# qgallouedec/deep_rl

Measured on NVIDIA B200. Metric: PPO env-steps/sec (rollout+update) CartPole-v1, higher is better.
Workload: dtype bf16

## Files before the change

### deep_rl_b200/_lib.py

```python
from __future__ import annotations

import ctypes as C
import os

import torch

from . import build as _build

_LIB = None

u8p, i32p, u32p, u64p, f32p, f64p = (C.c_void_p,) * 6


class EnvT(C.Structure):
    _fields_ = [("kind", C.c_int32), ("num_envs", C.c_int32), ("seed", C.c_uint64), ("env_gid0", C.c_uint32),
                ("max_episode_steps", C.c_int32), ("state", C.c_void_p), ("elapsed", C.c_void_p),
                ("ep_ret", C.c_void_p), ("ep_len", C.c_void_p)]


class EpLogT(C.Structure):
    _fields_ = [("count", C.c_void_p), ("sum_ret", C.c_void_p), ("sum_len", C.c_void_p), ("entries", C.c_void_p),
                ("cap", C.c_uint32)]


class NetT(C.Structure):
    _fields_ = [("obs_dim", C.c_int32), ("hidden", C.c_int32), ("num_actions", C.c_int32), ("obs_stride", C.c_int32)]


class RolloutBufT(C.Structure):
    _fields_ = [("obs", C.c_void_p), ("act", C.c_void_p), ("logp", C.c_void_p), ("val", C.c_void_p),
                ("rew", C.c_void_p), ("done", C.c_void_p), ("logits", C.c_void_p)]


class CommT(C.Structure):
    _fields_ = [("world", C.c_int32), ("rank", C.c_int32), ("peer", C.c_void_p * 8), ("seq", C.c_uint32),
                ("error_flag", C.c_void_p)]


class CtrlT(C.Structure):
    _fields_ = [("env_step", C.c_uint64), ("epoch_ctr", C.c_uint32), ("comm_seq", C.c_uint32), ("adam_step", C.c_int64),
                ("neg_step_size", C.c_float * 64), ("bc2_sqrt", C.c_float * 64)]


class PpoCoefT(C.Structure):
    _fields_ = [("clip_coef", C.c_float), ("ent_coef", C.c_float), ("vf_coef", C.c_float)]


SIGNATURES = {
    "drl_abi_version": (C.c_int, []),
    "drl_last_error": (C.c_char_p, []),
    "drl_env_obs_dim": (C.c_int, [C.c_int32]),
    "drl_env_num_actions": (C.c_int, [C.c_int32]),
    "drl_env_obs_stride": (C.c_int, [C.c_int32]),
    "drl_param_count": (C.c_int64, [C.POINTER(NetT)]),
    "drl_packed_count": (C.c_int64, [C.POINTER(NetT)]),
    "drl_record_width": (C.c_int, [C.POINTER(NetT)]),
    "drl_workspace_bytes": (C.c_size_t, [C.POINTER(NetT)]),
    "drl_env_reset": (C.c_int, [C.POINTER(EnvT), f32p, C.c_void_p]),
    "drl_env_observe": (C.c_int, [C.POINTER(EnvT), f32p, C.c_void_p]),
    "drl_env_step": (C.c_int, [C.POINTER(EnvT), C.c_uint64, i32p, f32p, f32p, u8p, C.POINTER(EpLogT), C.c_void_p]),
    "drl_pack_params": (C.c_int, [C.POINTER(NetT), f32p, f32p, C.c_void_p]),
    "drl_policy_forward": (C.c_int, [C.POINTER(NetT), f32p, f32p, C.c_int64, f32p, f32p, C.c_void_p]),
    "drl_sample": (C.c_int, [f32p, C.c_int64, C.c_int32, C.c_uint64, C.c_uint32, C.c_uint64, i32p, f32p, C.c_void_p]),
    "drl_rollout": (C.c_int, [C.POINTER(EnvT), C.POINTER(NetT), f32p, C.c_int32, C.c_uint64, C.POINTER(RolloutBufT),
                              C.POINTER(EpLogT), C.c_uint32, C.c_void_p]),
    "drl_gae": (C.c_int, [C.POINTER(RolloutBufT), C.POINTER(NetT), C.c_int32, C.c_int32, C.c_float, C.c_float, f32p,
                          f32p, f32p, C.c_void_p]),
    "drl_explained_variance": (C.c_int, [f32p, f32p, C.c_int64, f32p, C.c_void_p, C.c_size_t, C.c_void_p]),
    "drl_permutation": (C.c_int, [u32p, C.c_uint32, C.c_uint64, C.c_uint32, C.c_uint32, C.c_void_p]),
    "drl_adv_stats": (C.c_int, [C.POINTER(NetT), f32p, u32p, C.c_uint32, C.c_uint32, f32p, C.c_void_p, C.c_size_t,
                                C.c_void_p]),
    "drl_adv_stats_perm": (C.c_int, [C.POINTER(NetT), f32p, C.c_uint32, C.c_uint32, C.c_uint64, C.c_uint32, C.c_uint32, f32p,
                                     C.c_void_p, C.c_size_t, C.c_void_p]),
    "drl_ppo_minibatch_grad": (C.c_int, [C.POINTER(NetT), f32p, f32p, u32p, C.c_uint32, C.c_uint32, f32p,
                                         C.POINTER(PpoCoefT), f32p, f32p, C.c_void_p, C.c_size_t, C.c_uint32, C.c_void_p]),
    "drl_ppo_minibatch_update": (C.c_int, [C.POINTER(NetT), f32p, f32p, u32p, C.c_uint32, C.c_uint32, f32p, C.POINTER(PpoCoefT),
                                           f32p, f32p, f32p, f32p, C.c_int64, C.c_double, C.c_double, C.c_double, C.c_double,
                                           C.c_double, f32p, f32p, C.c_void_p, C.c_size_t, C.c_uint32, C.c_int32, C.c_void_p]),
    "drl_ppo_minibatch_update_dist": (C.c_int, [C.POINTER(NetT), f32p, f32p, u32p, C.c_uint32, C.c_uint32, f32p, C.POINTER(PpoCoefT),
                                                f32p, f32p, f32p, f32p, C.c_int64, C.c_double, C.c_double, C.c_double, C.c_double,
                                                C.c_double, f32p, f32p, C.c_void_p, C.c_size_t, C.c_uint32, C.POINTER(CommT),
                                                C.c_int32, C.c_void_p]),
    "drl_ctrl_set": (C.c_int, [C.c_void_p, C.c_uint64, C.c_uint32, C.c_uint32, C.c_int64, C.c_int32, C.c_double, C.c_double, C.c_double,
                               C.c_void_p]),
    "drl_rollout_ctl": (C.c_int, [C.POINTER(EnvT), C.POINTER(NetT), f32p, C.c_int32, C.c_void_p, C.POINTER(RolloutBufT),
                                  C.POINTER(EpLogT), C.c_uint32, C.c_void_p]),
    "drl_permutation_ctl": (C.c_int, [u32p, C.c_uint32, C.c_uint64, C.c_void_p, C.c_uint32, C.c_uint32, C.c_void_p]),
    "drl_adv_stats_perm_ctl": (C.c_int, [C.POINTER(NetT), f32p, C.c_uint32, C.c_uint32, C.c_uint64, C.c_void_p, C.c_uint32, C.c_uint32,
                                         f32p, C.c_void_p, C.c_size_t, C.c_void_p]),
    "drl_ppo_minibatch_update_ctl": (C.c_int, [C.POINTER(NetT), f32p, f32p, u32p, C.c_uint32, C.c_uint32, f32p, C.POINTER(PpoCoefT),
                                               f32p, f32p, f32p, f32p, C.c_void_p, C.c_int32, C.c_double, C.c_double, C.c_double,
                                               C.c_double, f32p, f32p, C.c_void_p, C.c_size_t, C.c_uint32, C.POINTER(CommT),
                                               C.c_int32, C.c_void_p]),
    "drl_comm_bytes": (C.c_size_t, [C.POINTER(NetT)]),
    "drl_comm_alloc": (C.c_int, [C.c_size_t, C.POINTER(C.c_void_p), C.c_void_p]),
    "drl_comm_open": (C.c_int, [C.c_void_p, C.POINTER(C.c_void_p)]),
    "drl_comm_close": (C.c_int, [C.c_void_p]),
    "drl_comm_free": (C.c_int, [C.c_void_p]),
    "drl_replay_sample_uniform": (C.c_int, [u32p, C.c_uint32, C.c_uint32, C.c_uint64, C.c_uint64, C.c_void_p]),
    "drl_replay_gather": (C.c_int, [f32p, i32p, f32p, u8p, u32p, C.c_uint32, C.c_int32, f32p, f32p, i32p, f32p, u8p, C.c_void_p]),
    "drl_replay_scratch_bytes": (C.c_size_t, [C.c_uint32]),
    "drl_replay_sample_priority": (C.c_int, [f32p, C.c_uint32, C.c_float, C.c_uint32, C.c_uint64, C.c_uint64, u32p, f32p, C.c_void_p,
                                             C.c_size_t, C.c_void_p]),
    "drl_replay_update_priorities": (C.c_int, [f32p, u32p, f32p, C.c_uint32, f32p, C.c_void_p]),
    "drl_reinforce_param_count": (C.c_int, []),
    "drl_reinforce_episodes": (C.c_int, [C.POINTER(EnvT), f32p, C.c_int32, C.c_uint64, f32p, u8p, f32p, u8p, i32p, u32p, C.POINTER(EpLogT),
                                         C.c_void_p]),
    "drl_reinforce_grad": (C.c_int, [f32p, f32p, u8p, f32p, i32p, u32p, C.c_int32, C.c_uint64, C.c_uint32, C.c_uint64, C.c_float, f32p, f32p,
                                     f32p, f32p, C.c_void_p]),
    "drl_adam_step": (C.c_int, [f32p, f32p, f32p, f32p, C.c_int64, C.c_int64, C.c_double, C.c_double, C.c_double, C.c_double, C.c_void_p]),
    "drl_selftest_umma": (C.c_int, [C.c_int32, C.c_int32, f32p, f32p, f32p, C.c_void_p]),
    "drl_selftest_tanh": (C.c_int, [f32p, f32p, C.c_int64, C.c_void_p]),
    "drl_clip_adam": (C.c_int, [C.POINTER(NetT), f32p, f32p, f32p, f32p, C.c_int64, C.c_double, C.c_double, C.c_double,
                                C.c_double, C.c_double, C.c_double, f32p, f32p, C.c_void_p]),
}


class DrlError(RuntimeError):
    pass


def lib_path() -> str:
    return _build.SO


ABI_VERSION = 2


def lib() -> C.CDLL:
    global _LIB
    if _LIB is None:
        path = _build.build_locked()
        L = C.CDLL(path)
        for name, (res, args) in SIGNATURES.items():
            fn = getattr(L, name)
            fn.restype, fn.argtypes = res, args
        if L.drl_abi_version() != ABI_VERSION:
            raise DrlError(f"libdrl_b200 ABI version {L.drl_abi_version()} != {ABI_VERSION}")
        _LIB = L
    return _LIB


def check(rc: int) -> None:
    if rc != 0:
        raise DrlError(f"libdrl_b200 error {rc}: {lib().drl_last_error().decode()}")


def require_cuda() -> None:
    if not torch.cuda.is_available():
        raise DrlError("deep_rl_b200 needs a CUDA device (B200, sm_100a); there is no CPU fallback")


def ptr(t) -> int:
    return 0 if t is None else t.data_ptr()


def stream_ptr() -> int:
    return torch.cuda.current_stream().cuda_stream
```

### deep_rl_b200/csrc/drl_pack.cuh

```cuda
#pragma once
#include <cuda_bf16.h>

#include "drl_common.cuh"

namespace drl {

int check_net(const drl_net_t* net);

template <int O, int A>
__device__ __forceinline__ void packed_store(float* __restrict__ packed, int i, float v) {
    using P = Packed<O, A>;
    const int net = i >= P::C_ACTOR ? 1 : 0;
    int r = i - net * P::C_ACTOR;
    if (r < H * O) {
        const int o = r / O, k = r % O;
        packed[P::W1T + (net * O + k) * H + perm_pos(o)] = v;
        packed[P::TC_W1 + (net * H + o) * P::OW + k] = __bfloat162float(__float2bfloat16_rn(v));
        __nv_bfloat16* w1b = reinterpret_cast<__nv_bfloat16*>(packed + P::TC_W1B) + net * (2 * H * 8);
        w1b[o * 8 + k] = __float2bfloat16_rn(v);
        w1b[H * 8 + o * 8 + k] = __float2bfloat16_rn(v);
        return;
    }
    r -= H * O;
    if (r < H) {
        packed[P::B1 + net * H + perm_pos(r)] = v;
        packed[P::TC_B1 + net * H + r] = __bfloat162float(__float2bfloat16_rn(v));
        reinterpret_cast<__nv_bfloat16*>(packed + P::TC_W1B)[net * (2 * H * 8) + r * 8 + O] = __float2bfloat16_rn(v);
        return;
    }
    r -= H;
    if (r < H * H) {
        const int o = r / H, k = r % H;
        packed[P::W2T + (net * H + k) * H + perm_pos(o)] = v;
        packed[P::W2P + (net * H + o) * H + perm_pos(k)] = v;
        unsigned char* tc = reinterpret_cast<unsigned char*>(packed + P::TC_W2);
        const int off = net * (H * H * 2) + o * 128 + ((((k >> 3) ^ (o & 7)) << 4)) + (k & 7) * 2;
        *reinterpret_cast<__nv_bfloat16*>(tc + off) = __float2bfloat16_rn(v);
        return;
    }
    r -= H * H;
    if (r < H) {
        packed[P::B2 + net * H + perm_pos(r)] = v;
        packed[P::TC_B2 + net * H + r] = v;
        return;
    }
    r -= H;
    const int nout = net == 0 ? A : 1;
    if (r < nout * H) {
        const int a = r / H, k = r % H;
        packed[P::W4 + (net * A + a) * H + perm_pos(k)] = v;
        packed[P::TC_W4 + (net == 0 ? a : A) * H + k] = v;
        return;
    }
    r -= nout * H;
    packed[P::B4 + net * A + r] = v;
    packed[P::TC_B4 + (net == 0 ? r : A)] = v;
}

constexpr int MAX_GRAD_CTAS = 160;
constexpr int MAX_MINIBATCHES = 16;
constexpr int STAT_PARTS = 512;
constexpr int LOSS_TERMS = 8;

struct WorkspaceLayout {
    size_t counters, stat_partials, cta_sumsq, loss_partials, grad_partials, debug, ev_partials, stage, total;
    int ppad;
};
inline WorkspaceLayout workspace_layout(int64_t P, int hidden = 64) {
    WorkspaceLayout w;
    w.ppad = (int)((P + 3) / 4 * 4);
    w.counters = 0;
    w.stat_partials = 64;
    w.cta_sumsq = w.stat_partials + sizeof(double) * MAX_MINIBATCHES * STAT_PARTS * 2;
    w.ev_partials = w.cta_sumsq + sizeof(double) * 1024;
    w.loss_partials = w.ev_partials + sizeof(double) * STAT_PARTS * 4;
    w.grad_partials = w.loss_partials + sizeof(float) * MAX_GRAD_CTAS * LOSS_TERMS;
    w.debug = (w.grad_partials + sizeof(float) * (size_t)MAX_GRAD_CTAS * w.ppad + 1023) / 1024 * 1024;
    w.stage = w.debug + 4096;
    w.total = w.stage + (hidden == 256 ? (size_t)2 * 2 * 4096 * 65536 : 0);
    return w;
}
inline size_t workspace_bytes_for(int64_t P, int hidden = 64) { return workspace_layout(P, hidden).total; }

}
```

### deep_rl_b200/csrc/drl_update.cuh

```cuda
#pragma once
#include "drl_common.cuh"

namespace drl {

constexpr int DRL_MAX_STEPS_PER_LAUNCH = 8;

struct AdamArgs {
    float* params; const float* grad; float* m; float* v; float* packed; float* norm_out;
    int P;
    float grad_scale, max_norm, beta2, om_beta1, om_beta2, eps, neg_step_size, bc2_sqrt;
};

struct TailArgs {
    int enabled;
    AdamArgs a;
    float* grad_out; float* loss_terms_out;
    double* cta_sumsq;
    uint32_t* ctr;
    int world, rank;
    unsigned char* peer[DRL_MAX_RANKS];
    uint32_t seq;
    int* error_flag;
    const drl_ctrl_t* ctrl;
    int ordinal;
    int nsteps;
    float neg_step_size_s[DRL_MAX_STEPS_PER_LAUNCH], bc2_sqrt_s[DRL_MAX_STEPS_PER_LAUNCH];
};

constexpr int FLAG_CTAS = 160;
struct CommLayout {
    size_t xgrad[2], flags[2], rank_stride, total;
};
__host__ __device__ inline CommLayout comm_layout(int64_t P) {
    CommLayout c;
    const size_t g = ((size_t)P * 4 + 255) / 256 * 256;
    c.rank_stride = g;
    c.xgrad[0] = 0; c.xgrad[1] = (size_t)DRL_MAX_RANKS * g;
    c.flags[0] = 2 * (size_t)DRL_MAX_RANKS * g; c.flags[1] = c.flags[0] + sizeof(uint32_t) * DRL_MAX_RANKS * FLAG_CTAS;
    c.total = c.flags[1] + sizeof(uint32_t) * DRL_MAX_RANKS * FLAG_CTAS;
    return c;
}

struct GradArgs {
    const float* packed;
    const float* rec;
    const uint32_t* idx;
    uint32_t mb_start, mb_count;
    const float* adv_stats;
    float clip_coef, ent_coef, vf_coef;
    float* grad_part;
    float* loss_part;
    int ppad;
    long long* dbg;
    TailArgs tail;
};

int launch_grad_reduce(const GradArgs& g, int grid, int P, float* grad_out, float* loss_terms_out, cudaStream_t st);

int launch_grad_tc(const drl_net_t* net, const GradArgs& g, int P, float* grad_out, float* loss_terms_out, cudaStream_t st,
                   int* grid_out = nullptr);
int launch_grad_tc_fused(const drl_net_t* net, GradArgs& g, cudaStream_t st);

}
```

### deep_rl_b200/csrc/gae_ops.cu

```cuda
#include "drl_pack.cuh"

namespace drl {

template <int OP, int RW>
__global__ void __launch_bounds__(128) gae_kernel(const float* __restrict__ rew, const uint8_t* __restrict__ done,
                                                   const float* __restrict__ val, const float* __restrict__ obs,
                                                   const uint8_t* __restrict__ act, const float* __restrict__ logp,
                                                   int T, int N, float gamma, float lam, float* __restrict__ adv,
                                                   float* __restrict__ ret, float* __restrict__ rec) {
    const int n = blockIdx.x * blockDim.x + threadIdx.x;
    if (n >= N) return;
    float last = 0.0f;
    float v1 = val[(size_t)T * N + n];
    adv[(size_t)T * N + n] = 0.0f;
    ret[(size_t)T * N + n] = 0.0f + v1;
    constexpr int GB = 8;
    for (int tb = T - 1; tb >= 0; tb -= GB) {
        float r_[GB], v_[GB], lp_[GB];
        uint8_t d_[GB], a_[GB];
        float4 o_[GB][OP / 4];
#pragma unroll
        for (int j = 0; j < GB; ++j) {
            const int t = tb - j;
            if (t >= 0) {
                const size_t i0 = (size_t)t * N + n, i1 = i0 + N;
                d_[j] = done[i1];
                r_[j] = rew[i1];
                v_[j] = val[i0];
                if (rec != nullptr) {
                    lp_[j] = logp[i0];
                    a_[j] = act[i0];
                    const float4* o4 = reinterpret_cast<const float4*>(obs + i0 * OP);
#pragma unroll
                    for (int q = 0; q < OP / 4; ++q) o_[j][q] = o4[q];
                }
            }
        }
#pragma unroll
        for (int j = 0; j < GB; ++j) {
            const int t = tb - j;
            if (t >= 0) {
                const size_t i0 = (size_t)t * N + n;
                const float d = (float)d_[j];
                const float v0 = v_[j];
                const float nd = 1.0f - d;
                const float a = gamma * nd;
                const float ll = lam * last;
                const float b = v1 + ll;
                const float c = a * b;
                const float dd = r_[j] + c;
                const float ad = dd - v0;
                adv[i0] = ad;
                ret[i0] = ad + v0;
                if (rec != nullptr) {
                    float4* r4 = reinterpret_cast<float4*>(rec + i0 * RW);
                    r4[0] = o_[j][0];
                    if (RW == 16) {
                        r4[1] = o_[j][OP / 4 - 1];
                        r4[2] = make_float4(0.f, 0.f, 0.f, 0.f);
                    }
                    r4[RW / 4 - 1] = make_float4(lp_[j], ad, v0, __int_as_float((int)a_[j]));
                }
                last = ad;
                v1 = v0;
            }
        }
    }
}

constexpr int PERM_ROUNDS = 6;

__device__ __forceinline__ uint32_t fmix32(uint32_t h) {
    h ^= h >> 16; h *= 0x85EBCA6Bu; h ^= h >> 13; h *= 0xC2B2AE35u; h ^= h >> 16;
    return h;
}

__device__ __forceinline__ uint32_t perm_index(uint32_t i, uint32_t B, uint32_t a, uint32_t b, const uint32_t (&keys)[8]) {
    uint32_t x = i;
    do {
        uint32_t lb = a, rb = b;
        uint32_t L = x >> rb, R = x & ((1u << rb) - 1u);
#pragma unroll
        for (uint32_t r = 0; r < PERM_ROUNDS; ++r) {
            const uint32_t nR = L ^ (fmix32(R ^ keys[r]) & ((1u << lb) - 1u));
            L = R;
            R = nR;
            const uint32_t t = lb; lb = rb; rb = t;
        }
        x = (L << rb) | R;
    } while (x >= B);
    return x;
}

__global__ void __launch_bounds__(256) permutation_kernel(uint32_t* __restrict__ idx, uint32_t B, uint32_t a, uint32_t b,
                                                           uint64_t seed, uint32_t epoch_ctr, uint32_t rank,
                                                           const drl_ctrl_t* __restrict__ ctrl) {
    if (ctrl != nullptr) epoch_ctr += ctrl->epoch_ctr;
    const uint4 k0 = philox_seeded(seed, epoch_ctr, rank, 0u, TAG_PERM);
    const uint4 k1 = philox_seeded(seed, epoch_ctr, rank, 1u, TAG_PERM);
    const uint32_t keys[8] = {k0.x, k0.y, k0.z, k0.w, k1.x, k1.y, k1.z, k1.w};
    const uint32_t stride = gridDim.x * blockDim.x;
    for (uint32_t i = blockIdx.x * blockDim.x + threadIdx.x; i < B; i += stride)
        idx[i] = perm_index(i, B, a, b, keys);
}

template <int RW>
__global__ void __launch_bounds__(256) adv_stats_kernel(const float* __restrict__ rec, const uint32_t* __restrict__ idx,
                                                         uint32_t B, uint32_t mb_size, float* __restrict__ stats_out,
                                                         double* __restrict__ partials, uint32_t* __restrict__ counter) {
    const uint32_t mb = blockIdx.y, part = blockIdx.x, nmb = gridDim.y, nparts = gridDim.x;
    const uint32_t lo = mb * mb_size;
    const uint32_t hi = min(B, lo + mb_size);
    double s = 0.0, ss = 0.0;
    const uint32_t step = nparts * 256u;
    uint32_t i = lo + part * 256u + threadIdx.x;
    for (; i + 3u * step < hi; i += 4u * step) {
        uint32_t sx[4];
#pragma unroll
        for (int j = 0; j < 4; ++j) sx[j] = idx ? __ldg(idx + i + j * step) : i + j * step;
        float av[4];
#pragma unroll
        for (int j = 0; j < 4; ++j) av[j] = __ldg(rec + (size_t)sx[j] * RW + (RW - 3));
#pragma unroll
        for (int j = 0; j < 4; ++j) { const double a = (double)av[j]; s += a; ss = fma(a, a, ss); }
    }
    for (; i < hi; i += step) {
        const uint32_t sidx = idx ? idx[i] : i;
        const double a = (double)rec[(size_t)sidx * RW + (RW - 3)];
        s += a;
        ss = fma(a, a, ss);
    }
    __shared__ double sh[2][8];
    __shared__ bool is_last;
    s = warp_sum(s);
    ss = warp_sum(ss);
    const int warp = threadIdx.x >> 5, lane = threadIdx.x & 31;
    if (lane == 0) { sh[0][warp] = s; sh[1][warp] = ss; }
    __syncthreads();
    if (threadIdx.x == 0) {
        double ts = 0.0, tss = 0.0;
        for (int w = 0; w < 8; ++w) { ts += sh[0][w]; tss += sh[1][w]; }
        partials[((size_t)mb * STAT_PARTS + part) * 2 + 0] = ts;
        partials[((size_t)mb * STAT_PARTS + part) * 2 + 1] = tss;
        __threadfence();
        const uint32_t done = atomicAdd(counter, 1u);
        is_last = (done == nmb * nparts - 1);
    }
    __syncthreads();
    if (is_last && threadIdx.x < nmb) {
        __threadfence();
        const uint32_t k = threadIdx.x;
        double ts = 0.0, tss = 0.0;
        for (uint32_t p = 0; p < nparts; ++p) {
            ts += __ldcg(&partials[((size_t)k * STAT_PARTS + p) * 2 + 0]);
            tss += __ldcg(&partials[((size_t)k * STAT_PARTS + p) * 2 + 1]);
        }
        const uint32_t klo = k * mb_size, khi = min(B, klo + mb_size);
        const double cnt = (double)(khi - klo);
        const double mean = ts / cnt;
        const double var = (tss - ts * mean) / (cnt - 1.0);
        stats_out[2 * k + 0] = (float)mean;
        stats_out[2 * k + 1] = (float)sqrt(var > 0.0 ? var : 0.0);
        if (k == 0) *counter = 0;
    }
}

constexpr int STATS_MAX_MB = 8;

__device__ __forceinline__ uint32_t perm_position(uint32_t s, uint32_t B, uint32_t a, uint32_t b, const uint32_t (&keys)[8]) {
    uint32_t x = s;
    do {
        uint32_t lb = a, rb = b;
        uint32_t L = x >> rb, R = x & ((1u << rb) - 1u);
#pragma unroll
        for (int r = PERM_ROUNDS - 1; r >= 0; --r) {
            const uint32_t t = lb; lb = rb; rb = t;
            const uint32_t R0 = L;
            const uint32_t L0 = R ^ (fmix32(R0 ^ keys[r]) & ((1u << lb) - 1u));
            L = L0; R = R0;
        }
        x = (L << rb) | R;
    } while (x >= B);
    return x;
}

__global__ void __launch_bounds__(256) adv_stats_perm_kernel(const float* __restrict__ adv, uint32_t B, uint32_t mb_size, uint32_t nmb,
                                                              uint32_t a, uint32_t b, uint64_t seed, uint32_t epoch_ctr, uint32_t rank,
                                                              float* __restrict__ stats_out, double* __restrict__ partials,
                                                              uint32_t* __restrict__ counter, const drl_ctrl_t* __restrict__ ctrl) {
    if (ctrl != nullptr) epoch_ctr += ctrl->epoch_ctr;
    const uint4 k0 = philox_seeded(seed, epoch_ctr, rank, 0u, TAG_PERM);
    const uint4 k1 = philox_seeded(seed, epoch_ctr, rank, 1u, TAG_PERM);
    const uint32_t keys[8] = {k0.x, k0.y, k0.z, k0.w, k1.x, k1.y, k1.z, k1.w};
    double sm_[STATS_MAX_MB], ss_[STATS_MAX_MB];
#pragma unroll
    for (int m = 0; m < STATS_MAX_MB; ++m) { sm_[m] = 0.0; ss_[m] = 0.0; }
    const uint32_t stride = gridDim.x * blockDim.x;
    for (uint32_t s = blockIdx.x * blockDim.x + threadIdx.x; s < B; s += stride) {
        const double v = (double)__ldg(adv + s);
        const uint32_t mb = perm_position(s, B, a, b, keys) / mb_size;
#pragma unroll
        for (int m = 0; m < STATS_MAX_MB; ++m)
            if (mb == (uint32_t)m) { sm_[m] += v; ss_[m] = fma(v, v, ss_[m]); }
    }
    __shared__ double sh[2][STATS_MAX_MB][8];
    __shared__ bool is_last;
    const int warp = threadIdx.x >> 5, lane = threadIdx.x & 31;
#pragma unroll
    for (int m = 0; m < STATS_MAX_MB; ++m) {
        const double t0 = warp_sum(sm_[m]), t1 = warp_sum(ss_[m]);
        if (lane == 0) { sh[0][m][warp] = t0; sh[1][m][warp] = t1; }
    }
    __syncthreads();
    if (threadIdx.x < 2 * STATS_MAX_MB) {
        const int which = threadIdx.x / STATS_MAX_MB, m = threadIdx.x % STATS_MAX_MB;
        double t = 0.0;
        for (int w = 0; w < 8; ++w) t += sh[which][m][w];
        partials[((size_t)m * STAT_PARTS + blockIdx.x) * 2 + which] = t;
    }
    __threadfence();
    __syncthreads();
    if (threadIdx.x == 0) {
        const uint32_t done = atomicAdd(counter, 1u);
        is_last = (done == gridDim.x - 1);
    }
    __syncthreads();
    if (is_last) {
        __threadfence();
        const uint32_t k = threadIdx.x >> 5;
        if (k < nmb) {
            double ts = 0.0, tss = 0.0;
            for (uint32_t p = threadIdx.x & 31; p < gridDim.x; p += 32) {
                ts += __ldcg(&partials[((size_t)k * STAT_PARTS + p) * 2 + 0]);
                tss += __ldcg(&partials[((size_t)k * STAT_PARTS + p) * 2 + 1]);
            }
            ts = warp_sum(ts);
            tss = warp_sum(tss);
            if ((threadIdx.x & 31) == 0) {
                const uint32_t klo = k * mb_size, khi = min(B, klo + mb_size);
                const double cnt = (double)(khi - klo);
                const double mean = ts / cnt;
                const double var = (tss - ts * mean) / (cnt - 1.0);
                stats_out[2 * k + 0] = (float)mean;
                stats_out[2 * k + 1] = (float)sqrt(var > 0.0 ? var : 0.0);
            }
        }
        __syncthreads();
        if (threadIdx.x == 0) *counter = 0;
    }
}

__global__ void __launch_bounds__(256) explained_variance_kernel(const float* __restrict__ values, const float* __restrict__ returns,
                                                                  int64_t n, float* __restrict__ out, double* __restrict__ partials,
                                                                  uint32_t* __restrict__ counter) {
    double acc[4] = {0.0, 0.0, 0.0, 0.0};
    const int64_t stride = (int64_t)gridDim.x * blockDim.x;
    for (int64_t i = (int64_t)blockIdx.x * blockDim.x + threadIdx.x; i < n; i += stride) {
        const float yf = __ldg(values + i), rf = __ldg(returns + i);
        const double y = (double)yf, d = (double)(yf - rf);
        acc[0] += y; acc[1] = fma(y, y, acc[1]); acc[2] += d; acc[3] = fma(d, d, acc[3]);
    }
    __shared__ double sh[4][8];
    __shared__ bool is_last;
    const int warp = threadIdx.x >> 5, lane = threadIdx.x & 31;
#pragma unroll
    for (int q = 0; q < 4; ++q) {
        const double t = warp_sum(acc[q]);
        if (lane == 0) sh[q][warp] = t;
    }
    __syncthreads();
    if (threadIdx.x < 4) {
        double t = 0.0;
        for (int w = 0; w < 8; ++w) t += sh[threadIdx.x][w];
        partials[(size_t)blockIdx.x * 4 + threadIdx.x] = t;
    }
    __threadfence();
    __syncthreads();
    if (threadIdx.x == 0) is_last = atomicAdd(counter, 1u) == gridDim.x - 1;
    __syncthreads();
    if (is_last && threadIdx.x < 32) {
        __threadfence();
        double t[4] = {0.0, 0.0, 0.0, 0.0};
        for (uint32_t p = threadIdx.x; p < gridDim.x; p += 32)
#pragma unroll
            for (int q = 0; q < 4; ++q) t[q] += __ldcg(&partials[(size_t)p * 4 + q]);
#pragma unroll
        for (int q = 0; q < 4; ++q) t[q] = warp_sum(t[q]);
        if (threadIdx.x == 0) {
            const double cnt = (double)n;
            const double var_y = (t[1] - t[0] * (t[0] / cnt)) / (cnt - 1.0);
            const double var_d = (t[3] - t[2] * (t[2] / cnt)) / (cnt - 1.0);
            out[0] = var_y == 0.0 ? __int_as_float(0x7FC00000) : (float)(1.0 - var_d / var_y);
            *counter = 0;
        }
    }
}

}

using namespace drl;

extern "C" {

int drl_gae(const drl_rollout_buf_t* buf, const drl_net_t* net, int32_t T, int32_t N, float gamma, float gae_lambda,
            float* adv_out, float* ret_out, float* rec_out, void* stream) {
    int rc = check_net(net);
    if (rc != DRL_OK) return rc;
    DRL_REQUIRE(buf && buf->rew && buf->done && buf->val && adv_out && ret_out, "drl_gae: NULL pointer");
    DRL_REQUIRE(T > 0 && N > 0, "drl_gae: T=%d N=%d", T, N);
    DRL_REQUIRE(rec_out == nullptr || (buf->obs && buf->act && buf->logp), "drl_gae: record packing needs obs/act/logp");
    const int blocks = (N + 127) / 128;
    cudaStream_t st = as_stream(stream);
    if (net->obs_stride == 4)
        gae_kernel<4, 8><<<blocks, 128, 0, st>>>(buf->rew, buf->done, buf->val, buf->obs, buf->act, buf->logp, T, N, gamma,
                                                gae_lambda, adv_out, ret_out, rec_out);
    else
        gae_kernel<8, 16><<<blocks, 128, 0, st>>>(buf->rew, buf->done, buf->val, buf->obs, buf->act, buf->logp, T, N, gamma,
                                                 gae_lambda, adv_out, ret_out, rec_out);
    DRL_LAUNCH_CHECK("gae_kernel");
    return DRL_OK;
}

int drl_explained_variance(const float* values, const float* returns, int64_t n, float* out, void* workspace,
                           size_t workspace_bytes, void* stream) {
    DRL_REQUIRE(values && returns && out && workspace, "drl_explained_variance: NULL pointer");
    DRL_REQUIRE(n >= 2, "drl_explained_variance: n=%lld", (long long)n);
    const WorkspaceLayout w = workspace_layout(0);
    DRL_REQUIRE(workspace_bytes >= w.total, "drl_explained_variance: workspace %zu < %zu bytes", workspace_bytes, w.total);
    uint32_t* counter = reinterpret_cast<uint32_t*>((char*)workspace + w.counters) + 12;
    double* partials = reinterpret_cast<double*>((char*)workspace + w.ev_partials);
    int64_t blocks = (n + 4095) / 4096;
    if (blocks > STAT_PARTS) blocks = STAT_PARTS;
    explained_variance_kernel<<<(int)blocks, 256, 0, as_stream(stream)>>>(values, returns, n, out, partials, counter);
    DRL_LAUNCH_CHECK("explained_variance_kernel");
    return DRL_OK;
}

static int permutation_impl(uint32_t* idx_out, uint32_t B, uint64_t seed, uint32_t epoch_ctr, uint32_t rank, void* stream,
                            const drl_ctrl_t* ctrl) {
    DRL_REQUIRE(idx_out, "drl_permutation: idx_out is NULL");
    DRL_REQUIRE(B > 0 && B <= 0x80000000u, "drl_permutation: B=%u out of range", B);
    DRL_REQUIRE(rank < (1u << 24), "drl_permutation: rank=%u out of range", rank);
    uint32_t k = 2;
    while (k < 32 && (1ull << k) < (unsigned long long)B) ++k;
    const uint32_t a = k / 2, b = k - a;
    long long blocks = ((long long)B + 2047) / 2048;
    const long long cap = (long long)sm_count() * 16;
    if (blocks > cap) blocks = cap;
    permutation_kernel<<<(int)blocks, 256, 0, as_stream(stream)>>>(idx_out, B, a, b, seed, epoch_ctr, rank, ctrl);
    DRL_LAUNCH_CHECK("permutation_kernel");
    return DRL_OK;
}
int drl_permutation(uint32_t* idx_out, uint32_t B, uint64_t seed, uint32_t epoch_ctr, uint32_t rank, void* stream) {
    return permutation_impl(idx_out, B, seed, epoch_ctr, rank, stream, nullptr);
}
int drl_permutation_ctl(uint32_t* idx_out, uint32_t B, uint64_t seed, const drl_ctrl_t* ctrl, uint32_t epoch_off, uint32_t rank,
                        void* stream) {
    DRL_REQUIRE(ctrl != nullptr, "drl_permutation_ctl: ctrl is NULL");
    return permutation_impl(idx_out, B, seed, epoch_off, rank, stream, ctrl);
}

int drl_adv_stats(const drl_net_t* net, const float* rec, const uint32_t* idx, uint32_t B, uint32_t mb_size,
                  float* stats_out, void* workspace, size_t workspace_bytes, void* stream) {
    int rc = check_net(net);
    if (rc != DRL_OK) return rc;
    DRL_REQUIRE(rec && stats_out && workspace, "drl_adv_stats: NULL pointer");
    DRL_REQUIRE(B > 0 && mb_size > 0, "drl_adv_stats: B=%u mb_size=%u", B, mb_size);
    const uint32_t nmb = (B + mb_size - 1) / mb_size;
    DRL_REQUIRE(nmb <= (uint32_t)MAX_MINIBATCHES, "drl_adv_stats: %u minibatches > %d", nmb, MAX_MINIBATCHES);
    const WorkspaceLayout w = workspace_layout(drl_param_count(net));
    DRL_REQUIRE(workspace_bytes >= w.total, "drl_adv_stats: workspace %zu < %zu bytes", workspace_bytes, w.total);
    uint32_t* counter = reinterpret_cast<uint32_t*>((char*)workspace + w.counters);
    double* partials = reinterpret_cast<double*>((char*)workspace + w.stat_partials);
    uint32_t nparts = (mb_size + 4095u) / 4096u;
    if (nparts > (uint32_t)STAT_PARTS) nparts = STAT_PARTS;
    if (nparts == 0) nparts = 1;
    dim3 grid(nparts, nmb);
    if (net->obs_dim <= 4) adv_stats_kernel<8><<<grid, 256, 0, as_stream(stream)>>>(rec, idx, B, mb_size, stats_out, partials, counter);
    else adv_stats_kernel<16><<<grid, 256, 0, as_stream(stream)>>>(rec, idx, B, mb_size, stats_out, partials, counter);
    DRL_LAUNCH_CHECK("adv_stats_kernel");
    return DRL_OK;
}

static int adv_stats_perm_impl(const drl_net_t* net, const float* adv, uint32_t B, uint32_t mb_size, uint64_t seed, uint32_t epoch_ctr,
                               uint32_t rank, float* stats_out, void* workspace, size_t workspace_bytes, void* stream,
                               const drl_ctrl_t* ctrl) {
    int rc = check_net(net);
    if (rc != DRL_OK) return rc;
    DRL_REQUIRE(adv && stats_out && workspace, "drl_adv_stats_perm: NULL pointer");
    DRL_REQUIRE(B > 0 && mb_size > 0 && B <= 0x80000000u, "drl_adv_stats_perm: B=%u mb_size=%u", B, mb_size);
    const uint32_t nmb = (B + mb_size - 1) / mb_size;
    if (nmb > (uint32_t)STATS_MAX_MB) { set_error("drl_adv_stats_perm: %u minibatches > %d (use drl_adv_stats)", nmb, STATS_MAX_MB); return DRL_ERR_UNSUPPORTED; }
    const WorkspaceLayout w = workspace_layout(drl_param_count(net));
    DRL_REQUIRE(workspace_bytes >= w.total, "drl_adv_stats_perm: workspace %zu < %zu bytes", workspace_bytes, w.total);
    uint32_t* counter = reinterpret_cast<uint32_t*>((char*)workspace + w.counters);
    double* partials = reinterpret_cast<double*>((char*)workspace + w.stat_partials);
    uint32_t k = 2;
    while (k < 32 && (1ull << k) < (unsigned long long)B) ++k;
    uint32_t blocks = (B + 2047u) / 2048u;
    if (blocks > (uint32_t)STAT_PARTS) blocks = STAT_PARTS;
    adv_stats_perm_kernel<<<blocks, 256, 0, as_stream(stream)>>>(adv, B, mb_size, nmb, k / 2, k - k / 2, seed, epoch_ctr, rank,
                                                                 stats_out, partials, counter, ctrl);
    DRL_LAUNCH_CHECK("adv_stats_perm_kernel");
    return DRL_OK;
}
int drl_adv_stats_perm(const drl_net_t* net, const float* adv, uint32_t B, uint32_t mb_size, uint64_t seed, uint32_t epoch_ctr,
                       uint32_t rank, float* stats_out, void* workspace, size_t workspace_bytes, void* stream) {
    return adv_stats_perm_impl(net, adv, B, mb_size, seed, epoch_ctr, rank, stats_out, workspace, workspace_bytes, stream, nullptr);
}
int drl_adv_stats_perm_ctl(const drl_net_t* net, const float* adv, uint32_t B, uint32_t mb_size, uint64_t seed, const drl_ctrl_t* ctrl,
                           uint32_t epoch_off, uint32_t rank, float* stats_out, void* workspace, size_t workspace_bytes, void* stream) {
    DRL_REQUIRE(ctrl != nullptr, "drl_adv_stats_perm_ctl: ctrl is NULL");
    return adv_stats_perm_impl(net, adv, B, mb_size, seed, epoch_off, rank, stats_out, workspace, workspace_bytes, stream, ctrl);
}

}
```

### deep_rl_b200/csrc/update_tc.cu

```cuda
#include "drl_pack.cuh"
#include "drl_tc_common.cuh"
#include "drl_update.cuh"

namespace drl {

constexpr uint32_t C_ZF = 0, C_DH = 128, C_W2 = 256, C_B2 = 384, C_W4 = 400, C_W1 = 416, TC_COLS = 512;

template <int O, int A>
struct TcSmem {
    using P = Packed<O, A>;
    static constexpr int W_BYTES = (P::TC_END - P::TC_W2) * 4;
    static constexpr int OFF_W = 0;
    static constexpr int OFF_H1 = (OFF_W + W_BYTES + 1023) / 1024 * 1024;
    static constexpr int OFF_H2 = OFF_H1 + 65536;
    static constexpr int OFF_DZ = OFF_H2 + 32768;
    static constexpr int OFF_DZ1 = OFF_DZ + 32768;
    static constexpr int OFF_OBS = OFF_DZ1 + 32768;
    static constexpr int OFF_DOUT = OFF_OBS + 12288;
    static constexpr int OFF_SCAL = OFF_DOUT + 4096;
    static constexpr int OFF_BAR = OFF_SCAL + 3 * 2048;
    static constexpr int OFF_XCH = OFF_BAR + 128;
    static constexpr int OFF_RED = OFF_XCH + 2 * 2 * 4 * 128 * 4;
    static constexpr int OFF_CTX = OFF_RED + 16 * 12 * 4;
    static constexpr int TOTAL = OFF_CTX + 512 + 1024;
    static_assert(TOTAL <= 232448, "exceeds the 227 KB of shared memory a CTA can opt in to");
};

#ifdef DRL_TC_STAMPS
#define TC_STAMP(ev) do { if (g.dbg != nullptr && blockIdx.x == 0 && lane == 0 && k < 12 && (warp == 0 || warp == TC_COMPUTE / 32)) g.dbg[(warp == 0 ? 0 : 256) + k * 16 + (ev)] = clock64(); } while (0)
#define TC_KSTAMP(n) do { if (g.dbg != nullptr && blockIdx.x == 0 && tid == 0) g.dbg[256 + ((n) >> 3) * 16 + 8 + ((n) & 7)] = clock64(); } while (0)
#else
#define TC_STAMP(ev) do { } while (0)
#define TC_KSTAMP(n) do { } while (0)
#endif

enum : uint32_t { BAR_FWD = 1, BAR_BWD = 2, BAR_W1 = 3, BAR_PAIR0 = 4, BAR_L1 = 12 };

constexpr int GRAD_TC_BLOCK = TC_THREADS + 32;
constexpr int RING = 3;

__device__ __forceinline__ uint32_t tc_sample_index(const GradArgs& g, uint32_t mb_start, uint32_t mb_count, uint32_t tile, uint32_t ntiles, int r) {
    const uint32_t pos = tile * TC_TILE + (uint32_t)r;
    if (tile >= ntiles || pos >= mb_count) return 0xFFFFFFFFu;
    const uint32_t i = mb_start + pos;
    return g.idx ? __ldg(g.idx + i) : i;
}

struct TailCtx {
    TailArgs tl;
    float* grad_part; float* loss_part; float* packed; long long* dbg;
    int ppad; uint32_t mb_count; float ent_coef, vf_coef;
};
static_assert(sizeof(TailCtx) <= 512, "TailCtx block");

template <int O, int A>
__device__ __noinline__ void tc_tail_step(const TailCtx* cx, uint32_t s, uint32_t nsteps, unsigned char* sm, uint64_t* bars) {
    using P = Packed<O, A>;
    using S = TcSmem<O, A>;
    const int tid = threadIdx.x, warp = tid >> 5, lane = tid & 31;
    const struct { long long* dbg; } g = {cx->dbg};
    (void)g;
    constexpr uint32_t BAR_TAIL = 13;
    const TailArgs& tl = cx->tl;
    const AdamArgs& ad = tl.a;
    const int PP = ad.P;
    float neg_step_size = tl.neg_step_size_s[s], bc2_sqrt = tl.bc2_sqrt_s[s];
    uint32_t seq = tl.seq + s;
    if (tl.ctrl != nullptr) {
        neg_step_size = tl.ctrl->neg_step_size[tl.ordinal + s];
        bc2_sqrt = tl.ctrl->bc2_sqrt[tl.ordinal + s];
        seq = tl.ctrl->comm_seq + (uint32_t)(tl.ordinal + s) + 1u;
    }
    float* const loss_terms_out = tl.loss_terms_out != nullptr ? tl.loss_terms_out + LOSS_TERMS * s : nullptr;
    const uint32_t bar_target = (s + 1u) * gridDim.x;
    const int nparts = gridDim.x;
    float* tred = reinterpret_cast<float*>(sm + S::OFF_H1);
    double* dred = reinterpret_cast<double*>(sm + S::OFF_H1 + 4096);
    float* sbc = reinterpret_cast<float*>(sm + S::OFF_H1 + 8192);
    auto grid_barrier = [&](uint32_t* ctr) {
        named_bar_sync(BAR_TAIL, TC_COMPUTE);
        if (tid == 0) {
            asm volatile("red.release.gpu.global.add.u32 [%0], 1;" ::"l"(ctr) : "memory");
            uint32_t seen;
            do {
                asm volatile("ld.acquire.gpu.global.u32 %0, [%1];" : "=r"(seen) : "l"(ctr) : "memory");
            } while (seen < bar_target);
        }
        named_bar_sync(BAR_TAIL, TC_COMPUTE);
    };
    grid_barrier(tl.ctr + 0);
    TC_KSTAMP(6);
    const int chunk = (PP + nparts - 1) / nparts;
    const int p_lo = blockIdx.x * chunk, p_hi = min(PP, p_lo + chunk);
    const int pl = tid & 63, sl = tid >> 6;
    const bool multi = tl.world > 1;
    const CommLayout cl = comm_layout(PP);
    const uint32_t gen = seq & 1u;
    double sq = 0.0;
    for (int p0 = p_lo; p0 < p_hi; p0 += 64) {
        const int p = p0 + pl;
        float a0 = 0.f, a1 = 0.f, a2 = 0.f, a3 = 0.f;
        if (p < p_hi) {
            static_assert(MAX_GRAD_CTAS <= 160, "fold is unrolled for at most 160 partials");
            float pv[20];
#pragma unroll
            for (int j = 0; j < 20; ++j) {
                const int c = sl + 8 * j;
                pv[j] = c < nparts ? __ldcg(cx->grad_part + (size_t)c * cx->ppad + p) : 0.0f;
            }
            bool rest = false;
#pragma unroll
            for (int gq = 0; gq < 5; ++gq) {
                const int c = sl + 32 * gq;
                if (!rest && c + 24 < nparts) {
                    a0 += pv[4 * gq]; a1 += pv[4 * gq + 1]; a2 += pv[4 * gq + 2]; a3 += pv[4 * gq + 3];
                } else {
                    rest = true;
#pragma unroll
                    for (int q = 0; q < 4; ++q)
                        if (c + 8 * q < nparts) a0 += pv[4 * gq + q];
                }
            }
        }
        tred[sl * 64 + pl] = (a0 + a1) + (a2 + a3);
        named_bar_sync(BAR_TAIL, TC_COMPUTE);
        if (sl == 0 && p < p_hi) {
            float t = tred[pl];
#pragma unroll
            for (int y = 1; y < 8; ++y) t += tred[y * 64 + pl];
            if (multi) {
                for (int rk = 0; rk < tl.world; ++rk)
                    reinterpret_cast<float*>(tl.peer[rk] + cl.xgrad[gen] + (size_t)tl.rank * cl.rank_stride)[p] = t;
            } else {
                tl.grad_out[p] = t;
                const double gs = (double)(t * ad.grad_scale);
                sq = fma(gs, gs, sq);
            }
        }
        named_bar_sync(BAR_TAIL, TC_COMPUTE);
    }
    TC_KSTAMP(7);
    if (multi) {
        if (sl == 0) __threadfence_system();
        named_bar_sync(BAR_TAIL, TC_COMPUTE);
        if (tid < tl.world) {
            __threadfence_system();
            *reinterpret_cast<volatile uint32_t*>(tl.peer[tid] + cl.flags[gen] + sizeof(uint32_t) * (tl.rank * FLAG_CTAS + blockIdx.x)) = seq;
            const volatile uint32_t* f = reinterpret_cast<const volatile uint32_t*>(tl.peer[tl.rank] + cl.flags[gen] +
                                                                                    sizeof(uint32_t) * (tid * FLAG_CTAS + blockIdx.x));
            const long long t0 = clock64();
            while (*f < seq) {
                if (clock64() - t0 > 40000000000ll) {
                    if (tl.error_flag) { *reinterpret_cast<volatile int*>(tl.error_flag) = 1; __threadfence(); }
                    break;
                }
            }
            __threadfence_system();
        }
        named_bar_sync(BAR_TAIL, TC_COMPUTE);
        const float* mine = reinterpret_cast<const float*>(tl.peer[tl.rank] + cl.xgrad[gen]);
        for (int p = p_lo + tid; p < p_hi; p += TC_COMPUTE) {
            float t = 0.0f;
            for (int rk = 0; rk < tl.world; ++rk)
                t += __ldcg(mine + (size_t)rk * (cl.rank_stride / sizeof(float)) + p);
            tl.grad_out[p] = t;
            const double gs = (double)(t * ad.grad_scale);
            sq = fma(gs, gs, sq);
        }
    }
    sq = warp_sum(sq);
    if (lane == 0) dred[warp] = sq;
    named_bar_sync(BAR_TAIL, TC_COMPUTE);
    if (tid == 0) {
        double t = 0.0;
        for (int wv = 0; wv < TC_COMPUTE / 32; ++wv) t += dred[wv];
        tl.cta_sumsq[blockIdx.x] = t;
    }
    TC_KSTAMP(8);
    const int p_first = p_lo + tid;
    float pre_m = 0.f, pre_v = 0.f, pre_w = 0.f;
    if (p_first < p_hi) { pre_m = ad.m[p_first]; pre_v = ad.v[p_first]; pre_w = ad.params[p_first]; }
    grid_barrier(tl.ctr + 2);
    TC_KSTAMP(9);
    if (warp == 0) {
        double tot = 0.0;
        for (int i = lane; i < nparts; i += 32) tot += __ldcg(tl.cta_sumsq + i);
        tot = warp_sum(tot);
        if (lane == 0) {
            const float norm = (float)sqrt(tot);
            const float cf = ad.max_norm / (norm + 1e-6f);
            sbc[0] = cf < 1.0f ? cf : 1.0f;
            if (blockIdx.x == 0 && ad.norm_out) *ad.norm_out = norm;
        }
    } else if (blockIdx.x == 0 && warp >= 1 && warp <= 5 && loss_terms_out != nullptr) {
        float t = 0.f;
        for (int c = lane; c < nparts; c += 32) t += __ldcg(cx->loss_part + c * LOSS_TERMS + (warp - 1));
        t = warp_sum(t);
        if (lane == 0) sbc[4 + warp - 1] = t;
    }
    named_bar_sync(BAR_TAIL, TC_COMPUTE);
    const float coef = sbc[0];
    const bool peer_lost = multi && tl.error_flag != nullptr && *reinterpret_cast<volatile int*>(tl.error_flag) != 0;
    for (int p = p_lo + tid; p < p_hi && !peer_lost; p += TC_COMPUTE) {
        const float gsc = (__ldcg(tl.grad_out + p) * ad.grad_scale) * coef;
        float m, v, wgt;
        if (p == p_first) { m = pre_m; v = pre_v; wgt = pre_w; }
        else { m = ad.m[p]; v = ad.v[p]; wgt = ad.params[p]; }
        m = m + ad.om_beta1 * (gsc - m);
        v = v * ad.beta2 + (ad.om_beta2 * gsc) * gsc;
        const float denom = sqrtf(v) / bc2_sqrt + ad.eps;
        wgt = wgt + (neg_step_size * m) / denom;
        ad.m[p] = m; ad.v[p] = v; ad.params[p] = wgt;
        if (ad.packed != nullptr) packed_store<O, A>(ad.packed, p, wgt);
    }
    TC_KSTAMP(10);
    if (blockIdx.x == 0 && tid == 0 && loss_terms_out != nullptr) {
        const float inv = 1.0f / (float)cx->mb_count;
        const float pg = sbc[4] * inv, vl = 0.5f * sbc[5] * inv, en = sbc[6] * inv;
        loss_terms_out[0] = pg - cx->ent_coef * en + vl * cx->vf_coef;
        loss_terms_out[1] = pg; loss_terms_out[2] = vl; loss_terms_out[3] = en;
        loss_terms_out[4] = sbc[7] * inv; loss_terms_out[5] = sbc[8] * inv;
        loss_terms_out[6] = 0.0f; loss_terms_out[7] = 0.0f;
    }
    if (s + 1 < nsteps) {
        grid_barrier(tl.ctr + 1);
        if (tid == 0) {
            asm volatile("fence.proxy.async;" ::: "memory");
            mbar_expect_tx(bars, (uint32_t)S::W_BYTES);
            const char* src = reinterpret_cast<const char*>(cx->packed + P::TC_W2);
            for (uint32_t off = 0; off < (uint32_t)S::W_BYTES; off += 16384u) {
                const uint32_t nb = (uint32_t)S::W_BYTES - off < 16384u ? (uint32_t)S::W_BYTES - off : 16384u;
                bulk_g2s(sm + S::OFF_W + off, src + off, nb, bars);
            }
        }
    } else if (tid == 0) {
        __threadfence();
        if (atomicAdd(tl.ctr + 3, 1u) == gridDim.x - 1) { tl.ctr[0] = 0u; tl.ctr[1] = 0u; tl.ctr[2] = 0u; tl.ctr[3] = 0u; }
    }
}

template <int O, int A, int OP, int RW>
__global__ void __launch_bounds__(GRAD_TC_BLOCK, 1) ppo_grad_tc_kernel(const __grid_constant__ GradArgs g) {
    using P = Packed<O, A>;
    using S = TcSmem<O, A>;
    constexpr int OW = P::OW;
    extern __shared__ unsigned char smem_raw[];
    unsigned char* sm = smem_raw + ((1024u - (smem_u32(smem_raw) & 1023u)) & 1023u);
    unsigned char* tW2 = sm + S::OFF_W;
    const float* sW1 = reinterpret_cast<const float*>(sm + S::OFF_W + 2 * H * H * 2);
    const float* sB1 = sW1 + 2 * H * OW;
    const float* sB2 = sB1 + 2 * H;
    const float* sW4 = sB2 + 2 * H;
    const float* sB4 = sW4 + (A + 1) * H;
    unsigned char* tW1B = reinterpret_cast<unsigned char*>(const_cast<float*>(sB4 + 4));
    unsigned char* tH1 = sm + S::OFF_H1;
    unsigned char* tH2 = sm + S::OFF_H2;
    unsigned char* tDZ = sm + S::OFF_DZ;
    unsigned char* tDZ1 = sm + S::OFF_DZ1;
    unsigned char* tOBS = sm + S::OFF_OBS;
    unsigned char* tDOUT = sm + S::OFF_DOUT;
    uint4* sSCAL = reinterpret_cast<uint4*>(sm + S::OFF_SCAL);
    uint64_t* bars = reinterpret_cast<uint64_t*>(sm + S::OFF_BAR);
    uint64_t* ring_full = bars + 7;
    uint64_t* ring_empty = bars + 7 + RING;
    uint32_t* slot = reinterpret_cast<uint32_t*>(bars + 7 + 2 * RING);
    float* xch = reinterpret_cast<float*>(sm + S::OFF_XCH);
    float* red = reinterpret_cast<float*>(sm + S::OFF_RED);

    const int tid = threadIdx.x, warp = tid >> 5, lane = tid & 31;
    const bool is_mma_warp = warp == TC_COMPUTE / 32;
    const bool is_loader_warp = warp == TC_COMPUTE / 32 + 1;
    const int rw = warp & 3, half = (warp >> 2) & 1, net = (warp >> 3) & 1;
    const int r = rw * 32 + lane;
    const int u0 = half * HU;
    const uint32_t nsteps = g.tail.enabled ? (uint32_t)g.tail.nsteps : 1u;
    const uint32_t ntiles = (g.mb_count + TC_TILE - 1) / TC_TILE;
    const uint32_t nmy = (ntiles - blockIdx.x + gridDim.x - 1) / gridDim.x;

    TC_KSTAMP(0);
    if (tid == 0) {
#pragma unroll
        for (int i = 0; i < 7; ++i) mbar_init(bars + i, 1);
#pragma unroll
        for (int i = 0; i < RING; ++i) { mbar_init(ring_full + i, 32); mbar_init(ring_empty + i, 1); }
        mbar_fence_init();
    }
    if (warp == 1) umma::tmem_alloc(slot, TC_COLS);
    if (tid == 64 && g.tail.enabled) {
        TailCtx* c = reinterpret_cast<TailCtx*>(sm + S::OFF_CTX);
        c->tl = g.tail;
        c->grad_part = g.grad_part; c->loss_part = g.loss_part; c->packed = const_cast<float*>(g.packed); c->dbg = g.dbg;
        c->ppad = g.ppad; c->mb_count = g.mb_count; c->ent_coef = g.ent_coef; c->vf_coef = g.vf_coef;
    }
    umma::fence_before_sync();
    __syncthreads();
    umma::fence_after_sync();
    if (tid == 0) {
        mbar_expect_tx(bars, (uint32_t)S::W_BYTES);
        const char* src = reinterpret_cast<const char*>(g.packed + P::TC_W2);
        for (uint32_t off = 0; off < (uint32_t)S::W_BYTES; off += 16384u) {
            const uint32_t n = (uint32_t)S::W_BYTES - off < 16384u ? (uint32_t)S::W_BYTES - off : 16384u;
            bulk_g2s(sm + S::OFF_W + off, src + off, n, bars);
        }
    }
    const uint32_t tmem = *slot;

    if (is_loader_warp) {
        uint32_t sidx[4];
#pragma unroll
        for (int q = 0; q < 4; ++q) sidx[q] = tc_sample_index(g, g.mb_start, g.mb_count, blockIdx.x, ntiles, lane + 32 * q);
        uint32_t b = 0, use_par = 0;
        for (uint32_t jg = 0; jg < nsteps * nmy; ++jg) {
            const uint32_t j = jg % nmy;
            float4 rv[4][OP / 4 + 1];
#pragma unroll
            for (int q = 0; q < 4; ++q) {
#pragma unroll
                for (int c = 0; c <= OP / 4; ++c) rv[q][c] = make_float4(0.f, 0.f, 0.f, 0.f);
                rv[q][OP / 4].w = __int_as_float(-1);
                if (sidx[q] != 0xFFFFFFFFu) {
                    const float4* r4 = reinterpret_cast<const float4*>(g.rec + (size_t)sidx[q] * RW);
#pragma unroll
                    for (int c = 0; c < OP / 4; ++c) rv[q][c] = __ldg(r4 + c);
                    rv[q][OP / 4] = __ldg(r4 + RW / 4 - 1);
                }
            }
            if (jg + 1 < nsteps * nmy) {
                const uint32_t jn = (jg + 1) % nmy, sn = (jg + 1) / nmy;
#pragma unroll
                for (int q = 0; q < 4; ++q)
                    sidx[q] = tc_sample_index(g, g.mb_start + sn * g.mb_count, g.mb_count, blockIdx.x + jn * gridDim.x, ntiles, lane + 32 * q);
            }
            (void)j;
            if (jg >= RING) mbar_wait(ring_empty + b, use_par ^ 1u);
            unsigned char* obst = tOBS + b * 4096;
#pragma unroll
            for (int q = 0; q < 4; ++q) {
                const int row = lane + 32 * q;
                float o16[16];
#pragma unroll
                for (int i = 0; i < 16; ++i) o16[i] = 0.0f;
#pragma unroll
                for (int i = 0; i < O; ++i) {
                    const float4 v4 = rv[q][i / 4];
                    const float x = (i & 3) == 0 ? v4.x : ((i & 3) == 1 ? v4.y : ((i & 3) == 2 ? v4.z : v4.w));
                    const float hi = __bfloat162float(__float2bfloat16_rn(x));
                    o16[i] = hi;
                    o16[8 + i] = x - hi;
                }
                o16[O] = 1.0f;
                umma::store_row_ns16(obst, TC_TILE, row, o16);
                sSCAL[b * TC_TILE + row] = make_uint4(__float_as_uint(rv[q][OP / 4].x), __float_as_uint(rv[q][OP / 4].y),
                                                      __float_as_uint(rv[q][OP / 4].z), __float_as_uint(rv[q][OP / 4].w));
            }
            umma::fence_proxy_async();
            mbar_arrive(ring_full + b);
            if (++b == RING) { b = 0; use_par ^= 1u; }
        }
        __syncthreads();
        return;
    }

    if (is_mma_warp) {
        const uint32_t aW2 = smem_u32(tW2), aH1 = smem_u32(tH1), aH2 = smem_u32(tH2), aDZ = smem_u32(tDZ);
        const uint32_t aOBS = smem_u32(tOBS), aDOUT = smem_u32(tDOUT), aDZ1 = smem_u32(tDZ1);
        constexpr uint32_t ID_FWD = umma::make_idesc(128, 64, false, false);
        constexpr uint32_t ID_DH1 = umma::make_idesc(128, 64, false, true);
        constexpr uint32_t ID_W2 = umma::make_idesc(128, 128, true, true);
        constexpr uint32_t ID_N16 = umma::make_idesc(128, 16, true, true);
        const uint32_t aW1B = smem_u32(tW1B);
        constexpr uint32_t ID_L1 = umma::make_idesc(128, 64, false, false);
        auto issue_l1 = [&](uint32_t slot_b) {
            const uint32_t obsb = aOBS + slot_b * 4096;
#pragma unroll
            for (int n2 = 0; n2 < 2; ++n2)
                umma::mma(tmem + C_ZF + n2 * 64, umma::make_desc(obsb, 2048, 128, umma::LAYOUT_NONE),
                          umma::make_desc(aW1B + n2 * 2048, 1024, 128, umma::LAYOUT_NONE), ID_L1, 0u);
            umma::commit(bars + 4);
        };
        auto issue_fwd = [&](uint32_t k) {
            const uint32_t h1b = aH1 + (k & 1u) * 32768;
#pragma unroll
            for (int n2 = 0; n2 < 2; ++n2)
#pragma unroll
                for (int kb = 0; kb < 4; ++kb)
                    umma::mma(tmem + C_ZF + n2 * 64, umma::make_desc(h1b + n2 * 16384 + kb * 32, 16, 1024, umma::LAYOUT_SW128),
                              umma::make_desc(aW2 + n2 * 8192 + kb * 32, 16, 1024, umma::LAYOUT_SW128), ID_FWD, kb > 0);
            umma::commit(bars + 1);
        };
        uint32_t bn = 0, bn_par = 0;
        uint32_t bc = 0;
        for (uint32_t s = 0; s < nsteps; ++s) {
        const uint32_t kbase = s * nmy;
        mbar_wait(bars, s & 1u);
        named_bar_sync(BAR_L1, TC_THREADS);
        mbar_wait(ring_full + bn, bn_par);
        umma::fence_after_sync();
        if (umma::elect_one()) issue_l1(bn);
        __syncwarp();
        if (++bn == RING) { bn = 0; bn_par ^= 1u; }
        named_bar_sync(BAR_FWD, TC_THREADS);
        umma::fence_after_sync();
        if (umma::elect_one()) issue_fwd(kbase);
        __syncwarp();
        for (uint32_t k = 0; k < nmy; ++k) {
            const uint32_t par = (kbase + k) & 1u, acc = k > 0 ? 1u : 0u;
            const uint32_t obsb = aOBS + bc * 4096;
            if (k + 1 < nmy) {
                named_bar_sync(BAR_L1, TC_THREADS);
                mbar_wait(ring_full + bn, bn_par);
                umma::fence_after_sync();
                if (umma::elect_one()) issue_l1(bn);
                __syncwarp();
                if (++bn == RING) { bn = 0; bn_par ^= 1u; }
            }
            named_bar_sync(BAR_BWD, TC_THREADS);
            umma::fence_after_sync();
            TC_STAMP(0);
            if (umma::elect_one()) {
#pragma unroll
                for (int n2 = 0; n2 < 2; ++n2)
#pragma unroll
                    for (int kb = 0; kb < 4; ++kb)
                        umma::mma(tmem + C_DH + n2 * 64, umma::make_desc(aDZ + n2 * 16384 + kb * 32, 16, 1024, umma::LAYOUT_SW128),
                                  umma::make_desc(aW2 + n2 * 8192 + kb * 2048, 8192, 1024, umma::LAYOUT_SW128), ID_DH1, kb > 0);
                umma::commit(bars + 2);
#ifdef DRL_TC_STAMPS
                if (g.dbg != nullptr && blockIdx.x == 0 && k < 12) g.dbg[256 + k * 16 + 6] = clock64();
#endif
            }
            __syncwarp();
            TC_STAMP(1);
            if (k + 1 < nmy) {
                named_bar_sync(BAR_FWD, TC_THREADS);
                umma::fence_after_sync();
                TC_STAMP(2);
                if (umma::elect_one()) issue_fwd(kbase + k + 1);
                __syncwarp();
                TC_STAMP(3);
            }
            if (umma::elect_one()) {
                const uint32_t h1b = aH1 + par * 32768;
#pragma unroll
                for (int kb = 0; kb < 8; ++kb)
                    umma::mma(tmem + C_W4, umma::make_desc(aH2 + kb * 2048, 16384, 1024, umma::LAYOUT_SW128),
                              umma::make_desc(aDOUT + kb * 256, 128, 2048, umma::LAYOUT_NONE), ID_N16, acc | (kb > 0));
                umma::commit(bars + 5);
#pragma unroll
                for (int kb = 0; kb < 8; ++kb)
                    umma::mma(tmem + C_W2, umma::make_desc(aDZ + kb * 2048, 16384, 1024, umma::LAYOUT_SW128),
                              umma::make_desc(h1b + kb * 2048, 16384, 1024, umma::LAYOUT_SW128), ID_W2, acc | (kb > 0));
#pragma unroll
                for (int kb = 0; kb < 8; ++kb)
                    umma::mma(tmem + C_B2, umma::make_desc(aDZ + kb * 2048, 16384, 1024, umma::LAYOUT_SW128),
                              umma::make_desc(obsb + kb * 256, 128, 2048, umma::LAYOUT_NONE), ID_N16, acc | (kb > 0));
                umma::commit(bars + 6);
            }
            __syncwarp();
            named_bar_sync(BAR_W1, TC_THREADS);
            umma::fence_after_sync();
            TC_STAMP(4);
            if (umma::elect_one()) {
#pragma unroll
                for (int kb = 0; kb < 8; ++kb)
                    umma::mma(tmem + C_W1, umma::make_desc(aDZ1 + kb * 2048, 16384, 1024, umma::LAYOUT_SW128),
                              umma::make_desc(obsb + kb * 256, 128, 2048, umma::LAYOUT_NONE), ID_N16, acc | (kb > 0));
                umma::commit(bars + 3);
                umma::commit(ring_empty + bc);
            }
            __syncwarp();
            TC_STAMP(5);
            if (++bc == RING) bc = 0;
        }
        }
        umma::fence_before_sync();
        __syncthreads();
        return;
    }

    const uint32_t trow = tmem + ((uint32_t)(rw * 32) << 16);
    const float inv_m = 1.0f / (float)g.mb_count;
    const int wrow0 = net == 0 ? 0 : A;
    const int nheads = net == 0 ? A : 1;
    uint32_t rb = 0, rb_par = 0;

    for (uint32_t s = 0; s < nsteps; ++s) {
    const uint32_t kbase = s * nmy;
    const float adv_mean = g.adv_stats[2 * s], adv_rstd = 1.0f / (g.adv_stats[2 * s + 1] + 1e-8f);
    float lsum[5] = {0.f, 0.f, 0.f, 0.f, 0.f};
    float gb4[4] = {0.f, 0.f, 0.f, 0.f};

    TC_KSTAMP(1);
    mbar_wait(bars, s & 1u);
    TC_KSTAMP(2);

    auto phase0 = [&](uint32_t k) {
        mbar_wait(bars + 4, k & 1u);
        umma::fence_after_sync();
        float h[HU];
        umma::ld32(trow + C_ZF + net * 64 + u0, h);
#pragma unroll
        for (int j = 0; j < HU; ++j) h[j] = tanh_mufu(h[j]);
        store_half_row_sw128(tH1 + (k & 1u) * 32768 + net * 16384, r, half * 4, h);
        umma::fence_proxy_async();
        umma::fence_before_sync();
        named_bar_arrive(BAR_FWD, TC_THREADS);
    };

    named_bar_arrive(BAR_L1, TC_THREADS);
    phase0(kbase);
    TC_KSTAMP(3);

    for (uint32_t k = 0; k < nmy; ++k) {
        const uint32_t par = (kbase + k) & 1u;

        TC_STAMP(0);
        mbar_wait(bars + 1, par);
        umma::fence_after_sync();
        TC_STAMP(1);
        {
            float h[HU];
            umma::ld32(trow + C_ZF + net * 64 + u0, h);
            if (k + 1 < nmy) {
                umma::fence_before_sync();
                named_bar_arrive(BAR_L1, TC_THREADS);
            }
            const float* b2 = sB2 + net * H + u0;
#pragma unroll
            for (int k4 = 0; k4 < HU / 4; ++k4) {
                const float4 bb = *reinterpret_cast<const float4*>(b2 + 4 * k4);
                h[4 * k4 + 0] = tanh_mufu(h[4 * k4 + 0] + bb.x);
                h[4 * k4 + 1] = tanh_mufu(h[4 * k4 + 1] + bb.y);
                h[4 * k4 + 2] = tanh_mufu(h[4 * k4 + 2] + bb.z);
                h[4 * k4 + 3] = tanh_mufu(h[4 * k4 + 3] + bb.w);
            }
            if (k > 0) mbar_wait(bars + 5, par ^ 1u);
            store_half_row_sw128(tH2 + net * 16384, r, half * 4, h);

            float ps[A];
#pragma unroll
            for (int a = 0; a < A; ++a) {
                ps[a] = 0.0f;
                if (a < nheads) {
                    const float* w = sW4 + (wrow0 + a) * H + u0;
                    float s0 = 0.f, s1 = 0.f, s2 = 0.f, s3 = 0.f;
#pragma unroll
                    for (int k4 = 0; k4 < HU / 4; ++k4) {
                        const float4 ww = *reinterpret_cast<const float4*>(w + 4 * k4);
                        s0 = fmaf(h[4 * k4 + 0], ww.x, s0);
                        s1 = fmaf(h[4 * k4 + 1], ww.y, s1);
                        s2 = fmaf(h[4 * k4 + 2], ww.z, s2);
                        s3 = fmaf(h[4 * k4 + 3], ww.w, s3);
                    }
                    ps[a] = (s0 + s1) + (s2 + s3);
                    xch[((net * 2 + half) * 4 + a) * TC_TILE + r] = ps[a];
                }
            }
            TC_STAMP(2);
            named_bar_sync(BAR_PAIR0 + net * 4 + rw, 64);
            TC_STAMP(3);
            float out[A];
#pragma unroll
            for (int a = 0; a < A; ++a) {
                out[a] = 0.0f;
                if (a < nheads) {
                    const float po = xch[((net * 2 + (half ^ 1)) * 4 + a) * TC_TILE + r];
                    const float lo = half == 0 ? ps[a] : po, hi = half == 0 ? po : ps[a];
                    out[a] = (lo + hi) + sB4[wrow0 + a];
                }
            }
            float d[A];
#pragma unroll
            for (int a = 0; a < A; ++a) d[a] = 0.0f;
            mbar_wait(ring_full + rb, rb_par);
            const uint4 sc = sSCAL[rb * TC_TILE + r];
            const float rc_logp_old = __uint_as_float(sc.x), rc_adv = __uint_as_float(sc.y), rc_val_old = __uint_as_float(sc.z);
            const int rc_act = (int)sc.w;
            if (rc_act >= 0) {
                if (net == 0) {
                    float m = out[0];
#pragma unroll
                    for (int a = 1; a < A; ++a) m = fmaxf(m, out[a]);
                    float se = 0.f;
#pragma unroll
                    for (int a = 0; a < A; ++a) se += __expf(out[a] - m);
                    const float lse = m + __logf(se);
                    float lp[A], p[A];
                    float ent = 0.f, new_logp = 0.f;
#pragma unroll
                    for (int a = 0; a < A; ++a) {
                        lp[a] = out[a] - lse;
                        p[a] = __expf(lp[a]);
                        ent -= p[a] * lp[a];
                        if (a == rc_act) new_logp = lp[a];
                    }
                    const float nadv = (rc_adv - adv_mean) * adv_rstd;
                    const float logratio = new_logp - rc_logp_old;
                    const float ratio = __expf(logratio);
                    const float pg1 = -nadv * ratio;
                    const float pg2 = -nadv * fminf(fmaxf(ratio, 1.0f - g.clip_coef), 1.0f + g.clip_coef);
                    const float dpg = pg1 >= pg2 ? pg1 : 0.0f;
                    if (half == 0) {
                        lsum[0] += fmaxf(pg1, pg2);
                        lsum[2] += ent;
                        lsum[3] += (ratio - 1.0f) - logratio;
                        lsum[4] += fabsf(ratio - 1.0f) > g.clip_coef ? 1.0f : 0.0f;
                    }
#pragma unroll
                    for (int a = 0; a < A; ++a) {
                        const float onehot = a == rc_act ? 1.0f : 0.0f;
                        d[a] = inv_m * (dpg * (onehot - p[a]) + g.ent_coef * p[a] * (lp[a] + ent));
                        if (half == 0) gb4[a] += d[a];
                    }
                } else {
                    const float v = out[0];
                    const float ret = rc_adv + rc_val_old;
                    const float vd = v - ret;
                    const float vu = vd * vd;
                    const float vdiff = v - rc_val_old;
                    const float vc = rc_val_old + fminf(fmaxf(vdiff, -g.clip_coef), g.clip_coef);
                    const float vcd = vc - ret;
                    const float vcl = vcd * vcd;
                    const float gcl = (vdiff >= -g.clip_coef && vdiff <= g.clip_coef) ? vcd : 0.0f;
                    const float gv = vu > vcl ? vd : (vcl > vu ? gcl : 0.5f * (vd + gcl));
                    d[0] = g.vf_coef * gv * inv_m;
                    if (half == 0) { lsum[1] += fmaxf(vu, vcl); gb4[3] += d[0]; }
                }
            }
            if (half == 0) {
                uint4 q = make_uint4(0u, 0u, 0u, 0u);
                if (net == 0) {
                    q.x = umma::pack_bf16(d[0], d[1]);
                    if constexpr (A > 2) q.y = umma::pack_bf16(d[2], 0.0f);
                } else {
                    q.x = umma::pack_bf16(d[0], 0.0f);
                }
                *reinterpret_cast<uint4*>(tDOUT + (size_t)net * TC_TILE * 16 + (size_t)r * 16) = q;
            }
#pragma unroll
            for (int k4 = 0; k4 < HU / 4; ++k4) {
                float dh[4] = {0.f, 0.f, 0.f, 0.f};
#pragma unroll
                for (int a = 0; a < A; ++a) {
                    if (a < nheads) {
                        const float4 ww = *reinterpret_cast<const float4*>(sW4 + (wrow0 + a) * H + u0 + 4 * k4);
                        dh[0] = fmaf(d[a], ww.x, dh[0]); dh[1] = fmaf(d[a], ww.y, dh[1]);
                        dh[2] = fmaf(d[a], ww.z, dh[2]); dh[3] = fmaf(d[a], ww.w, dh[3]);
                    }
                }
#pragma unroll
                for (int j = 0; j < 4; ++j) h[4 * k4 + j] = dh[j] * fmaf(-h[4 * k4 + j], h[4 * k4 + j], 1.0f);
            }
            TC_STAMP(4);
            TC_STAMP(5);
            if (k > 0) mbar_wait(bars + 6, par ^ 1u);
            store_half_row_sw128(tDZ + net * 16384, r, half * 4, h);
        }
        umma::fence_proxy_async();
        umma::fence_before_sync();
        named_bar_arrive(BAR_BWD, TC_THREADS);
        TC_STAMP(6);

        if (k + 1 < nmy) {
            phase0(kbase + k + 1);
        }

        TC_STAMP(7);
        {
            const unsigned char* h1row = tH1 + par * 32768 + net * 16384;
            uint4 hq[4];
#pragma unroll
            for (int c = 0; c < 4; ++c) hq[c] = *reinterpret_cast<const uint4*>(h1row + umma::sw128_off(r, half * 4 + c));
            TC_STAMP(10);
            mbar_wait(bars + 2, par);
            TC_STAMP(11);
            if (k > 0) mbar_wait(bars + 3, par ^ 1u);
            umma::fence_after_sync();
            TC_STAMP(8);
            float dh[HU];
            umma::ld32(trow + C_DH + net * 64 + u0, dh);
            unsigned char* dzrow = tDZ1 + net * 16384;
#pragma unroll
            for (int c = 0; c < 4; ++c) {
                const uint4 q = hq[c];
                const float hv[8] = {umma::bf16_lo(q.x), umma::bf16_hi(q.x), umma::bf16_lo(q.y), umma::bf16_hi(q.y),
                                     umma::bf16_lo(q.z), umma::bf16_hi(q.z), umma::bf16_lo(q.w), umma::bf16_hi(q.w)};
                float z[8];
#pragma unroll
                for (int j = 0; j < 8; ++j) z[j] = dh[8 * c + j] * fmaf(-hv[j], hv[j], 1.0f);
                uint4 o4;
                o4.x = umma::pack_bf16(z[0], z[1]); o4.y = umma::pack_bf16(z[2], z[3]);
                o4.z = umma::pack_bf16(z[4], z[5]); o4.w = umma::pack_bf16(z[6], z[7]);
                *reinterpret_cast<uint4*>(dzrow + umma::sw128_off(r, half * 4 + c)) = o4;
            }
        }
        umma::fence_proxy_async();
        umma::fence_before_sync();
        named_bar_arrive(BAR_W1, TC_THREADS);
        TC_STAMP(9);
        if (++rb == RING) { rb = 0; rb_par ^= 1u; }
    }
    mbar_wait(bars + 3, (kbase + nmy - 1) & 1u);
    mbar_wait(bars + 5, (kbase + nmy - 1) & 1u);
    mbar_wait(bars + 6, (kbase + nmy - 1) & 1u);
    umma::fence_after_sync();
    TC_KSTAMP(4);

    float* stage = reinterpret_cast<float*>(sm + S::OFF_H1);
    float* part = g.grad_part + (size_t)blockIdx.x * g.ppad;
    const int no = r >> 6, o = r & 63;
    constexpr int W2_OFF = H * O + H;
    if (warp < 4) {
        const int base = no * P::C_ACTOR;
        float v16[16];
        umma::ld16(trow + C_B2, v16);
        stage[base + H * O + H + H * H + o] = v16[O];
        umma::ld16(trow + C_W1, v16);
#pragma unroll
        for (int i = 0; i < O; ++i) stage[base + o * O + i] = v16[i] + v16[8 + i];
        stage[base + H * O + o] = v16[O];
        umma::ld16(trow + C_W4, v16);
        if (no == 0) {
#pragma unroll
            for (int a = 0; a < A; ++a) stage[P::C_NET + a * H + o] = v16[a];
        } else {
            stage[P::C_ACTOR + P::C_NET + o] = v16[8];
        }
    }
    if (no == net) {
        float v[HU];
        umma::ld32(trow + C_W2 + net * 64 + u0, v);
        float* dst = stage + net * P::C_ACTOR + W2_OFF + o * H;
#pragma unroll
        for (int i = 0; i < HU; ++i) dst[(u0 + i) ^ (o & 31)] = v[i];
    }
    {
        float vals[9] = {lsum[0], lsum[1], lsum[2], lsum[3], lsum[4], gb4[0], gb4[1], gb4[2], gb4[3]};
#pragma unroll
        for (int q = 0; q < 9; ++q) {
            const float sv = warp_sum(vals[q]);
            if (lane == 0) red[warp * 12 + q] = sv;
        }
    }
    umma::fence_before_sync();
    named_bar_sync(13, TC_COMPUTE);
    if (tid < 9) {
        float sv = 0.0f;
#pragma unroll
        for (int w = 0; w < TC_COMPUTE / 32; ++w) sv += red[w * 12 + tid];
        if (tid < 5) g.loss_part[blockIdx.x * LOSS_TERMS + tid] = sv;
        else if (tid - 5 < A) stage[P::C_NET + A * H + (tid - 5)] = sv;
        else if (tid == 8) stage[P::C_ACTOR + P::C_NET + H] = sv;
    }
    named_bar_sync(13, TC_COMPUTE);
    for (int i = tid; i < P::C_ALL; i += TC_COMPUTE) {
        const int nb = i >= P::C_ACTOR ? 1 : 0;
        const int w = i - nb * P::C_ACTOR - W2_OFF;
        int src = i;
        if (w >= 0 && w < H * H) src = i - (w & 63) + ((w & 63) ^ ((w >> 6) & 31));
        part[i] = stage[src];
    }
    TC_KSTAMP(5);
    if (g.tail.enabled) tc_tail_step<O, A>(reinterpret_cast<const TailCtx*>(sm + S::OFF_CTX), s, nsteps, sm, bars);
    }
    umma::fence_before_sync();
    __syncthreads();
    if (warp == 1) umma::tmem_dealloc(tmem, TC_COLS);
}

template <int O, int A, int OP, int RW>
static int launch_tc_fused(GradArgs& g, cudaStream_t st) {
    const int smem = TcSmem<O, A>::TOTAL;
    DRL_CUDA(cudaFuncSetAttribute(ppo_grad_tc_kernel<O, A, OP, RW>, cudaFuncAttributeMaxDynamicSharedMemorySize, smem));
    const uint32_t ntiles = (g.mb_count + TC_TILE - 1) / TC_TILE;
    int grid = sm_count();
    if (grid > MAX_GRAD_CTAS) grid = MAX_GRAD_CTAS;
    if ((uint32_t)grid > ntiles) grid = (int)ntiles;
    void* args[] = {&g};
    DRL_CUDA(cudaLaunchCooperativeKernel((const void*)ppo_grad_tc_kernel<O, A, OP, RW>, dim3(grid), dim3(GRAD_TC_BLOCK), args, (size_t)smem, st));
    return DRL_OK;
}

int launch_grad_tc_fused(const drl_net_t* net, GradArgs& g, cudaStream_t st) {
    if (net->obs_dim == 4) return launch_tc_fused<4, 2, 4, 8>(g, st);
    if (net->obs_dim == 2) return launch_tc_fused<2, 3, 4, 8>(g, st);
    return launch_tc_fused<6, 3, 8, 16>(g, st);
}

template <int O, int A, int OP, int RW>
static int launch_tc(const GradArgs& g, int P, float* grad_out, float* loss_terms_out, cudaStream_t st, int* grid_out) {
    const int smem = TcSmem<O, A>::TOTAL;
    DRL_CUDA(cudaFuncSetAttribute(ppo_grad_tc_kernel<O, A, OP, RW>, cudaFuncAttributeMaxDynamicSharedMemorySize, smem));
    const uint32_t ntiles = (g.mb_count + TC_TILE - 1) / TC_TILE;
    int grid = sm_count();
    if (grid > MAX_GRAD_CTAS) grid = MAX_GRAD_CTAS;
    if ((uint32_t)grid > ntiles) grid = (int)ntiles;
    ppo_grad_tc_kernel<O, A, OP, RW><<<grid, GRAD_TC_BLOCK, smem, st>>>(g);
    DRL_LAUNCH_CHECK("ppo_grad_tc_kernel");
    if (grid_out != nullptr) { *grid_out = grid; return DRL_OK; }
    return launch_grad_reduce(g, grid, P, grad_out, loss_terms_out, st);
}

int launch_grad_tc(const drl_net_t* net, const GradArgs& g, int P, float* grad_out, float* loss_terms_out, cudaStream_t st,
                   int* grid_out) {
    if (net->obs_dim == 4) return launch_tc<4, 2, 4, 8>(g, P, grad_out, loss_terms_out, st, grid_out);
    if (net->obs_dim == 2) return launch_tc<2, 3, 4, 8>(g, P, grad_out, loss_terms_out, st, grid_out);
    return launch_tc<6, 3, 8, 16>(g, P, grad_out, loss_terms_out, st, grid_out);
}

}
```

### deep_rl_b200/ppo.py

```python
from __future__ import annotations

import argparse
import contextlib
import ctypes as C
from dataclasses import dataclass
from typing import Dict, Optional

import torch

from . import _lib, dist as _dist
from .agent import ActorCritic
from .envs import VecEnv


@dataclass
class PPOConfig:
    env_id: str = "CartPole-v1"
    total_timesteps: int = 20_000
    num_steps: int = 128
    update_epochs: int = 4
    gamma: float = 0.99
    gae_lambda: float = 0.95
    learning_rate: float = 2.5e-4
    clip_coef: float = 0.2
    ent_coef: float = 0.01
    vf_coef: float = 0.5
    max_grad_norm: float = 0.5
    seed: int = 1
    num_envs: int = 1
    hidden: int = 64
    num_minibatches: int = 4
    anneal_lr: bool = True
    rollout_precision: str = "auto"
    overlap_streams: bool = True
    global_adv_stats: bool = False
    grad_allreduce: str = "peer"
    update_precision: str = "auto"
    debug_logits: bool = False
    steps_per_launch: int = 0
    cuda_graph: bool = True

    def resolved_update_precision(self) -> str:
        if self.update_precision == "auto":
            return "bf16" if (self.num_envs >= 2048 or self.hidden != 64) else "fp32"
        return self.update_precision

    def resolved_rollout_precision(self) -> str:
        return self.resolved_update_precision() if self.rollout_precision == "auto" else self.rollout_precision

    @property
    def batch_size(self) -> int:
        return self.num_envs * self.num_steps

    @property
    def minibatch_size(self) -> int:
        return self.batch_size // self.num_minibatches

    def num_updates(self, world: int = 1) -> int:
        return self.total_timesteps // (self.batch_size * world)


class _Phase:

    def __init__(self, tr: "PPOTrainer", name: str):
        self.tr, self.name = tr, name

    def __enter__(self):
        if self.tr.timing:
            self.t0 = torch.cuda.Event(enable_timing=True)
            self.t1 = torch.cuda.Event(enable_timing=True)
            self.t0.record()
        return self

    def __exit__(self, *exc):
        if self.tr.timing:
            self.t1.record()
            self.tr.phase_events.setdefault(self.name, []).append((self.t0, self.t1))
        return False


class MetricsRead:

    def __init__(self, tr: "PPOTrainer", host_terms: torch.Tensor, log_read):
        self.tr, self.host_terms, self.log_read = tr, host_terms, log_read
        self.d2h_bytes = 36 + tr.env.log.last_d2h_bytes

    def result(self) -> Dict[str, object]:
        n, sum_ret, sum_len, e, lost = self.log_read.result()
        lt = self.host_terms.tolist()
        return {"loss": lt[0], "pg_loss": lt[1], "v_loss": lt[2], "entropy": lt[3], "approx_kl": lt[4], "clipfrac": lt[5],
                "grad_norm": lt[8], "episodes": n, "episodes_dropped": max(0, n - self.tr.env.log.cap) + max(0, min(n, self.tr.env.log.cap) - len(e)),
                "mean_return": (sum_ret / n) if n else float("nan"), "mean_length": (sum_len / n) if n else float("nan"),
                "episode_log": {"step": e["step"], "env": e["env"], "ret": e["ret"], "len": e["len"]}}


class PPOTrainer:

    def __init__(self, cfg: PPOConfig, rank: int = 0, world: int = 1, device: Optional[torch.device] = None,
                 agent: Optional[ActorCritic] = None):
        _lib.require_cuda()
        self.cfg, self.rank, self.world = cfg, int(rank), int(world)
        self.L = _lib.lib()
        self.device = torch.device(device if device is not None else f"cuda:{torch.cuda.current_device()}")
        N, T = cfg.num_envs, cfg.num_steps
        self.env = VecEnv(cfg.env_id, num_envs=N, seed=cfg.seed, env_gid0=self.rank * N, device=self.device)
        if agent is None:
            torch.manual_seed(cfg.seed)
            agent = ActorCritic(self.env, hidden=cfg.hidden, device=self.device, sample_seed=cfg.seed)
        self.agent = agent
        self.net = agent.net
        OP = self.env.obs_stride
        dev = self.device
        f32, u8 = torch.float32, torch.uint8
        self.observations = torch.zeros((T + 1, N, OP), dtype=f32, device=dev)
        self.actions = torch.zeros((T + 1, N), dtype=u8, device=dev)
        self.log_probs = torch.zeros((T + 1, N), dtype=f32, device=dev)
        self.values = torch.zeros((T + 1, N), dtype=f32, device=dev)
        self.rewards = torch.zeros((T + 1, N), dtype=f32, device=dev)
        self.dones = torch.zeros((T + 1, N), dtype=u8, device=dev)
        self.advantages = torch.zeros((T + 1, N), dtype=f32, device=dev)
        self.returns = torch.zeros((T + 1, N), dtype=f32, device=dev)
        self.logits = torch.zeros((T, N, self.env.num_actions), dtype=f32, device=dev) if cfg.debug_logits else None
        self.buf = _lib.RolloutBufT(self.observations.data_ptr(), self.actions.data_ptr(), self.log_probs.data_ptr(),
                                    self.values.data_ptr(), self.rewards.data_ptr(), self.dones.data_ptr(),
                                    _lib.ptr(self.logits))
        B = cfg.batch_size
        self.RW = self.L.drl_record_width(C.byref(self.net))
        self.records = torch.zeros((B, self.RW), dtype=f32, device=dev)
        self.n_mb = (B + cfg.minibatch_size - 1) // cfg.minibatch_size
        self.idx = torch.zeros((cfg.update_epochs, B), dtype=torch.int32, device=dev)
        self.adv_stats = torch.zeros((cfg.update_epochs, self.n_mb, 2), dtype=f32, device=dev)
        self.side = torch.cuda.Stream(device=dev) if cfg.overlap_streams else None
        self._ev_gae = torch.cuda.Event()
        self._ev_stats = [torch.cuda.Event() for _ in range(cfg.update_epochs)]
        self._perms_scheduled = False
        self._merge_stats = bool(cfg.global_adv_stats and self.world > 1 and torch.distributed.is_available()
                                 and torch.distributed.is_initialized())
        M_ = cfg.minibatch_size
        self._mb_counts = torch.tensor([[min(M_, B - k * M_) for k in range(self.n_mb)]] * cfg.update_epochs, dtype=torch.float64, device=dev)
        P = agent.flat_params.numel()
        self.grad = torch.zeros(P, dtype=f32, device=dev)
        self.exp_avg = torch.zeros(P, dtype=f32, device=dev)
        self.exp_avg_sq = torch.zeros(P, dtype=f32, device=dev)
        n_rows = cfg.update_epochs * self.n_mb
        self._terms_and_norm = torch.zeros(n_rows * 8 + 1, dtype=f32, device=dev)
        self.loss_terms = self._terms_and_norm[: n_rows * 8].view(n_rows, 8)
        self.grad_norm = self._terms_and_norm[n_rows * 8:]
        self._h_terms = torch.zeros(9, dtype=f32).pin_memory()
        self._h_terms_ring = [torch.zeros(9, dtype=f32).pin_memory() for _ in range(2)]
        self._h_flip = 0
        self.ws_bytes = int(self.L.drl_workspace_bytes(C.byref(self.net)))
        self.workspace = torch.zeros(self.ws_bytes, dtype=u8, device=dev)
        self.coef = _lib.PpoCoefT(cfg.clip_coef, cfg.ent_coef, cfg.vf_coef)
        if cfg.hidden != 64 and "fp32" in (cfg.resolved_update_precision(), cfg.resolved_rollout_precision()):
            raise ValueError(f"hidden={cfg.hidden} exists on the tensor-core (bf16) path only")
        if cfg.update_precision not in ("auto", "bf16", "fp32"):
            raise ValueError(f"update_precision={cfg.update_precision!r}")
        if cfg.rollout_precision not in ("auto", "bf16", "fp32"):
            raise ValueError(f"rollout_precision={cfg.rollout_precision!r}")
        self.update_precision = cfg.resolved_update_precision()
        self.rollout_precision = cfg.resolved_rollout_precision()
        self.grad_flags = 1 if self.update_precision == "bf16" else 0
        self.rollout_flags = 1 if self.rollout_precision == "bf16" else 0
        self._ev_out = torch.zeros(1, dtype=f32, device=dev)
        self.adam_step = 0
        self.update_idx = 0
        self.global_step = 0
        self.env.reset()
        self.kernel_launches = 0
        self.fused_step = cfg.hidden == 64
        self.peer = None
        if (self.world > 1 and cfg.grad_allreduce == "peer" and self.grad_flags == 1 and cfg.hidden == 64
                and torch.distributed.is_available() and torch.distributed.is_initialized()):
            self.peer = _dist.PeerComm(self.net, self.rank, self.world, dev)
        equal = B % cfg.minibatch_size == 0
        self.mb_per_launch = 1
        if self.grad_flags == 1 and cfg.hidden == 64 and equal and (self.world == 1 or self.peer is not None):
            want = cfg.steps_per_launch if cfg.steps_per_launch > 0 else (self.n_mb if cfg.minibatch_size <= (1 << 19) else 1)
            self.mb_per_launch = max(1, min(want, self.n_mb, 8))
            while self.n_mb % self.mb_per_launch:
                self.mb_per_launch -= 1
        self.timing = False
        self.phase_events: Dict[str, list] = {}
        self.ctrl = torch.zeros(C.sizeof(_lib.CtrlT), dtype=u8, device=dev)
        self._graph = None
        self._graph_launches = 0
        self._graph_warm = 0
        n_opt = cfg.update_epochs * self.n_mb
        self.graph_ok = bool(cfg.cuda_graph and self.grad_flags == 1 and cfg.hidden == 64 and self.n_mb <= 8 and n_opt <= 64 and not self._merge_stats
                             and (self.world == 1 or self.peer is not None))

    def phase_ms(self) -> Dict[str, Dict[str, float]]:
        torch.cuda.synchronize()
        out = {}
        for name, evs in self.phase_events.items():
            ms = [a.elapsed_time(b) for a, b in evs]
            out[name] = {"calls": len(ms), "total_ms": float(sum(ms)), "mean_ms": float(sum(ms) / max(1, len(ms)))}
        return out

    def learning_rate(self, update: int, num_updates: int) -> float:
        if not self.cfg.anneal_lr:
            return self.cfg.learning_rate
        return (1.0 - update / num_updates) * self.cfg.learning_rate

    def rollout(self, ctl: bool = False) -> None:
        cfg = self.cfg
        with _Phase(self, "rollout"):
            if ctl:
                _lib.check(self.L.drl_rollout_ctl(C.byref(self.env.struct), C.byref(self.net), self.agent.packed.data_ptr(),
                                                  cfg.num_steps, self.ctrl.data_ptr(), C.byref(self.buf),
                                                  C.byref(self.env.log.struct), self.rollout_flags, _lib.stream_ptr()))
            else:
                _lib.check(self.L.drl_rollout(C.byref(self.env.struct), C.byref(self.net), self.agent.packed.data_ptr(),
                                              cfg.num_steps, self.env.step_count, C.byref(self.buf),
                                              C.byref(self.env.log.struct), self.rollout_flags, _lib.stream_ptr()))
        self.env.step_count += cfg.num_steps
        self.global_step += cfg.num_steps * cfg.num_envs * self.world
        self.kernel_launches += 1

    def compute_gae(self) -> None:
        cfg = self.cfg
        with _Phase(self, "gae"):
            _lib.check(self.L.drl_gae(C.byref(self.buf), C.byref(self.net), cfg.num_steps, cfg.num_envs, cfg.gamma,
                                      cfg.gae_lambda, self.advantages.data_ptr(), self.returns.data_ptr(),
                                      self.records.data_ptr(), _lib.stream_ptr()))
        self.kernel_launches += 1

    def _side(self):
        return torch.cuda.stream(self.side) if self.side is not None else contextlib.nullcontext()

    def schedule_permutations(self, ctl: bool = False) -> None:
        cfg = self.cfg
        if self.side is not None:
            self.side.wait_stream(torch.cuda.current_stream())
        with self._side():
            st = _lib.stream_ptr()
            for epoch in range(cfg.update_epochs):
                epoch_ctr = self.update_idx * cfg.update_epochs + epoch
                with _Phase(self, "permutation"):
                    if ctl:
                        _lib.check(self.L.drl_permutation_ctl(self.idx[epoch].data_ptr(), cfg.batch_size, cfg.seed, self.ctrl.data_ptr(),
                                                              epoch, self.rank, st))
                    else:
                        _lib.check(self.L.drl_permutation(self.idx[epoch].data_ptr(), cfg.batch_size, cfg.seed, epoch_ctr, self.rank, st))
        self.kernel_launches += cfg.update_epochs
        self._perms_scheduled = True

    def schedule_adv_stats(self, ctl: bool = False) -> None:
        cfg = self.cfg
        B, M = cfg.batch_size, cfg.minibatch_size
        net = C.byref(self.net)
        if self.side is not None:
            self._ev_gae.record()
            self.side.wait_event(self._ev_gae)
        with self._side():
            st = _lib.stream_ptr()
            for epoch in range(cfg.update_epochs):
                epoch_ctr = self.update_idx * cfg.update_epochs + epoch
                with _Phase(self, "adv_stats"):
                    if ctl:
                        _lib.check(self.L.drl_adv_stats_perm_ctl(net, self.advantages.data_ptr(), B, M, cfg.seed, self.ctrl.data_ptr(), epoch,
                                                                 self.rank, self.adv_stats[epoch].data_ptr(), self.workspace.data_ptr(),
                                                                 self.ws_bytes, st))
                    elif self.n_mb <= 8:
                        _lib.check(self.L.drl_adv_stats_perm(net, self.advantages.data_ptr(), B, M, cfg.seed, epoch_ctr, self.rank,
                                                             self.adv_stats[epoch].data_ptr(), self.workspace.data_ptr(),
                                                             self.ws_bytes, st))
                    else:
                        _lib.check(self.L.drl_adv_stats(net, self.records.data_ptr(), self.idx[epoch].data_ptr(), B, M,
                                                        self.adv_stats[epoch].data_ptr(), self.workspace.data_ptr(),
                                                        self.ws_bytes, st))
                if self.side is not None and not self._merge_stats:
                    self._ev_stats[epoch].record()
            if self._merge_stats:
                _dist.merge_minibatch_stats(self.adv_stats, self._mb_counts)
                if self.side is not None:
                    for ev in self._ev_stats:
                        ev.record()
        self.kernel_launches += cfg.update_epochs

    def optimize(self, lr: float, ctl: bool = False) -> None:
        cfg = self.cfg
        B, M = cfg.batch_size, cfg.minibatch_size
        net = C.byref(self.net)
        if self.world > 1 and self.peer is None and not (torch.distributed.is_available() and torch.distributed.is_initialized()):
            raise _lib.DrlError("world > 1 needs an initialised torch.distributed process group for the gradient all-reduce "
                                "(deep_rl_b200.dist.init_from_env); without it the gradient would only be scaled by 1/world")
        if not self._perms_scheduled:
            self.schedule_permutations(ctl)
        self._perms_scheduled = False
        self.schedule_adv_stats(ctl)
        st = _lib.stream_ptr()
        for epoch in range(cfg.update_epochs):
            if self.side is not None:
                torch.cuda.current_stream().wait_event(self._ev_stats[epoch])
            idx_ptr = self.idx[epoch].data_ptr()
            stats_ptr = self.adv_stats[epoch].data_ptr()
            for k in range(0, self.n_mb, self.mb_per_launch):
                start = k * M
                count = min(M, B - start)
                row = epoch * self.n_mb + k
                ns = self.mb_per_launch
                if ctl:
                    self.adam_step += ns
                    if self.peer is not None:
                        for _ in range(ns):
                            self.peer.next()
                    with _Phase(self, "minibatch_grad"):
                        _lib.check(self.L.drl_ppo_minibatch_update_ctl(
                            net, self.agent.packed.data_ptr(), self.records.data_ptr(), idx_ptr, start, count,
                            stats_ptr + 8 * k, C.byref(self.coef), self.agent.flat_params.data_ptr(),
                            self.grad.data_ptr(), self.exp_avg.data_ptr(), self.exp_avg_sq.data_ptr(), self.ctrl.data_ptr(), row,
                            0.9, 0.999, 1e-5, cfg.max_grad_norm, self.loss_terms.data_ptr() + 32 * row,
                            self.grad_norm.data_ptr(), self.workspace.data_ptr(), self.ws_bytes, self.grad_flags,
                            C.byref(self.peer.struct) if self.peer is not None else None, ns, st))
                    self.kernel_launches += 1
                    continue
                if self.peer is not None:
                    first_step = self.adam_step + 1
                    self.adam_step += ns
                    comm = self.peer.next()
                    for _ in range(ns - 1):
                        self.peer.next()
                    comm.seq = self.peer.seq - ns + 1
                    with _Phase(self, "minibatch_grad"):
                        _lib.check(self.L.drl_ppo_minibatch_update_dist(
                            net, self.agent.packed.data_ptr(), self.records.data_ptr(), idx_ptr, start, count,
                            stats_ptr + 8 * k, C.byref(self.coef), self.agent.flat_params.data_ptr(),
                            self.grad.data_ptr(), self.exp_avg.data_ptr(), self.exp_avg_sq.data_ptr(), first_step, lr,
                            0.9, 0.999, 1e-5, cfg.max_grad_norm, self.loss_terms.data_ptr() + 32 * row,
                            self.grad_norm.data_ptr(), self.workspace.data_ptr(), self.ws_bytes, self.grad_flags,
                            C.byref(comm), ns, st))
                    comm.seq = self.peer.seq
                    self.kernel_launches += 1
                    continue
                if self.world == 1 and self.fused_step:
                    first_step = self.adam_step + 1
                    self.adam_step += ns
                    with _Phase(self, "minibatch_grad"):
                        _lib.check(self.L.drl_ppo_minibatch_update(
                            net, self.agent.packed.data_ptr(), self.records.data_ptr(), idx_ptr, start, count,
                            stats_ptr + 8 * k, C.byref(self.coef), self.agent.flat_params.data_ptr(),
                            self.grad.data_ptr(), self.exp_avg.data_ptr(), self.exp_avg_sq.data_ptr(), first_step, lr,
                            0.9, 0.999, 1e-5, cfg.max_grad_norm, self.loss_terms.data_ptr() + 32 * row,
                            self.grad_norm.data_ptr(), self.workspace.data_ptr(), self.ws_bytes, self.grad_flags, ns, st))
                    self.kernel_launches += 1 if self.grad_flags == 1 else 2
                    continue
                with _Phase(self, "minibatch_grad"):
                    _lib.check(self.L.drl_ppo_minibatch_grad(
                        net, self.agent.packed.data_ptr(), self.records.data_ptr(), idx_ptr, start, count,
                        stats_ptr + 8 * k, C.byref(self.coef), self.grad.data_ptr(),
                        self.loss_terms.data_ptr() + 32 * row, self.workspace.data_ptr(), self.ws_bytes, self.grad_flags, st))
                if self.world > 1:
                    with _Phase(self, "allreduce"):
                        _dist.all_reduce_sum(self.grad)
                self.adam_step += 1
                with _Phase(self, "clip_adam"):
                    _lib.check(self.L.drl_clip_adam(net, self.agent.flat_params.data_ptr(), self.grad.data_ptr(),
                                                    self.exp_avg.data_ptr(), self.exp_avg_sq.data_ptr(), self.adam_step, lr,
                                                    0.9, 0.999, 1e-5, cfg.max_grad_norm, 1.0 / self.world,
                                                    self.agent.packed.data_ptr(), self.grad_norm.data_ptr(), st))
                self.kernel_launches += 3

    def _issue_update(self, lr: float, ctl: bool) -> None:
        self.schedule_permutations(ctl)
        self.rollout(ctl)
        self.compute_gae()
        self.optimize(lr, ctl)

    def update(self, num_updates: Optional[int] = None) -> None:
        nu = num_updates if num_updates is not None else max(1, self.cfg.num_updates(self.world))
        lr = self.learning_rate(self.update_idx, nu)
        use_ctl = self.graph_ok and not self.timing
        if not use_ctl:
            self._issue_update(lr, False)
        else:
            cfg = self.cfg
            n_opt = cfg.update_epochs * self.n_mb
            _lib.check(self.L.drl_ctrl_set(self.ctrl.data_ptr(), self.env.step_count, self.update_idx * cfg.update_epochs,
                                           self.peer.seq if self.peer is not None else 0, self.adam_step, n_opt, lr, 0.9, 0.999,
                                           _lib.stream_ptr()))
            if self._graph is None and self._graph_warm >= 2:
                self._capture_graph(lr)
            if self._graph is not None:
                self._graph.replay()
                self._advance_host_counters(n_opt)
                self.kernel_launches += self._graph_launches
            else:
                self._graph_warm += 1
                self._issue_update(lr, True)
            self.kernel_launches += 1
        self.update_idx += 1
        self.agent.mark_packed_current()

    def _advance_host_counters(self, n_opt: int) -> None:
        cfg = self.cfg
        self.env.step_count += cfg.num_steps
        self.global_step += cfg.num_steps * cfg.num_envs * self.world
        self.adam_step += n_opt
        if self.peer is not None:
            self.peer.seq += n_opt

    def _capture_graph(self, lr: float) -> None:
        snap = (self.env.step_count, self.global_step, self.adam_step, self.kernel_launches, self.peer.seq if self.peer is not None else 0,
                self._perms_scheduled)
        torch.cuda.synchronize()
        g = torch.cuda.CUDAGraph()
        with torch.cuda.graph(g):
            self._issue_update(lr, True)
        self._graph_launches = self.kernel_launches - snap[3]
        self.env.step_count, self.global_step, self.adam_step, self.kernel_launches = snap[0], snap[1], snap[2], snap[3]
        if self.peer is not None:
            self.peer.seq = snap[4]
        self._perms_scheduled = False
        self._graph = g

    def metrics(self, with_episode_log: bool = True) -> Dict[str, float]:
        self._h_terms.copy_(self._d_terms_src(), non_blocking=True)
        if with_episode_log == "arrays":
            n, sum_ret, sum_len, entries = self.env.log.drain_arrays()
        else:
            n, sum_ret, sum_len, entries = self.env.log.drain(with_entries=with_episode_log)
        lt = self._h_terms.tolist()
        self.check_peers()
        return {"loss": lt[0], "pg_loss": lt[1], "v_loss": lt[2], "entropy": lt[3], "approx_kl": lt[4],
                "clipfrac": lt[5], "grad_norm": lt[8], "episodes": n, "episodes_dropped": max(0, n - self.env.log.cap),
                "mean_return": (sum_ret / n) if n else float("nan"), "mean_length": (sum_len / n) if n else float("nan"),
                "episode_log": entries}

    def metrics_async(self) -> "MetricsRead":
        host = self._h_terms_ring[self._h_flip]
        self._h_flip ^= 1
        host.copy_(self._d_terms_src(), non_blocking=True)
        return MetricsRead(self, host, self.env.log.read_async())

    def check_peers(self) -> None:
        if self.peer is not None and int(self.peer.error_flag.item()) != 0:
            raise _lib.DrlError("a peer rank did not arrive at the in-kernel all-reduce within the timeout; "
                                "optimizer steps have been skipped since")

    def _d_terms_src(self) -> torch.Tensor:
        return self._terms_and_norm[-9:]

    def state_dict(self) -> Dict[str, object]:
        e = self.env
        self.check_peers()
        return {"model": {k: v.detach().cpu().clone() for k, v in self.agent.state_dict().items()},
                "exp_avg": self.exp_avg.cpu().clone(), "exp_avg_sq": self.exp_avg_sq.cpu().clone(),
                "adam_step": self.adam_step, "update_idx": self.update_idx, "global_step": self.global_step,
                "env": {"state": e.state.cpu().clone(), "elapsed": e.elapsed.cpu().clone(), "ep_ret": e.ep_ret.cpu().clone(),
                        "ep_len": e.ep_len.cpu().clone(), "step_count": e.step_count},
                "carry": {"rewards0": self.rewards[0].cpu().clone(), "dones0": self.dones[0].cpu().clone()},
                "config": self._resume_key()}

    def _resume_key(self) -> Dict[str, object]:
        c = self.cfg
        return {"env_id": c.env_id, "num_envs": c.num_envs, "num_steps": c.num_steps, "seed": c.seed, "hidden": c.hidden,
                "rank": self.rank, "world": self.world, "update_precision": self.update_precision,
                "rollout_precision": self.rollout_precision}

    def load_state_dict(self, sd: Dict[str, object]) -> None:
        c, mine = sd["config"], self._resume_key()
        diff = {k: (c.get(k), v) for k, v in mine.items() if c.get(k) != v}
        if diff:
            raise ValueError(f"checkpoint does not match this trainer (checkpoint, trainer): {diff}")
        self.agent.load_state_dict(sd["model"])
        self.agent.sync()
        self.exp_avg.copy_(sd["exp_avg"])
        self.exp_avg_sq.copy_(sd["exp_avg_sq"])
        self.adam_step, self.update_idx, self.global_step = int(sd["adam_step"]), int(sd["update_idx"]), int(sd["global_step"])
        e, se = self.env, sd["env"]
        e.state.copy_(se["state"]); e.elapsed.copy_(se["elapsed"]); e.ep_ret.copy_(se["ep_ret"]); e.ep_len.copy_(se["ep_len"])
        e.step_count = int(se["step_count"])
        self.rewards[0].copy_(sd["carry"]["rewards0"])
        self.dones[0].copy_(sd["carry"]["dones0"])
        self._perms_scheduled = False

    def explained_variance(self) -> float:
        _lib.check(self.L.drl_explained_variance(self.values.data_ptr(), self.returns.data_ptr(), self.values.numel(),
                                                 self._ev_out.data_ptr(), self.workspace.data_ptr(), self.ws_bytes,
                                                 _lib.stream_ptr()))
        return float(self._ev_out.item())


def train(cfg: PPOConfig, quiet: bool = False, rank: int = 0, world: int = 1) -> PPOTrainer:
    tr = PPOTrainer(cfg, rank=rank, world=world)
    nu = cfg.num_updates(world)
    per_vec_step = cfg.num_envs * world
    for _ in range(nu):
        tr.update(nu)
        m = tr.metrics()
        if not quiet and rank == 0:
            if cfg.num_envs * world <= 16:
                for step, env_gid, ret, _len in m["episode_log"]:
                    print(f"global_step={step * per_vec_step + env_gid}, episodic_return={ret:.2f}")
            elif m["episodes"]:
                print(f"global_step={tr.global_step}, episodic_return={m['mean_return']:.2f} "
                      f"(mean of {m['episodes']} episodes)")
    return tr


def main(argv=None) -> None:
    p = argparse.ArgumentParser(description="PPO on device-resident classic-control envs (B200)")
    d = PPOConfig()
    p.add_argument("--env-id", default=d.env_id)
    p.add_argument("--total-timesteps", type=int, default=d.total_timesteps)
    p.add_argument("--num-steps", type=int, default=d.num_steps)
    p.add_argument("--num-envs", type=int, default=d.num_envs)
    p.add_argument("--update-epochs", type=int, default=d.update_epochs)
    p.add_argument("--learning-rate", type=float, default=d.learning_rate)
    p.add_argument("--seed", type=int, default=d.seed)
    a = p.parse_args(argv)
    rank, world = _dist.init_from_env()
    cfg = PPOConfig(env_id=a.env_id, total_timesteps=a.total_timesteps, num_steps=a.num_steps, num_envs=a.num_envs,
                    update_epochs=a.update_epochs, learning_rate=a.learning_rate, seed=a.seed)
    train(cfg, rank=rank, world=world)
    _dist.shutdown()


if __name__ == "__main__":
    main()
```

### include/drl_b200.h

```cpp
#ifndef DRL_B200_H
#define DRL_B200_H

#include <stddef.h>
#include <stdint.h>

#ifdef __cplusplus
extern "C" {
#endif

#define DRL_ABI_VERSION 2

enum { DRL_ENV_CARTPOLE = 0, DRL_ENV_ACROBOT = 1, DRL_ENV_MOUNTAINCAR = 2 };
enum { DRL_OK = 0, DRL_ERR_ARG = -1, DRL_ERR_UNSUPPORTED = -2, DRL_ERR_CUDA = -3 };

typedef struct {
    int32_t  kind;
    int32_t  num_envs;
    uint64_t seed;
    uint32_t env_gid0;
    int32_t  max_episode_steps;
    double*  state;
    int32_t* elapsed;
    float*   ep_ret;
    int32_t* ep_len;
} drl_env_t;

typedef struct {
    uint64_t step;
    uint32_t env;
    float    ret;
    int32_t  len;
    uint32_t pad;
} drl_ep_entry_t;
typedef struct {
    uint32_t*       count;
    double*         sum_ret;
    double*         sum_len;
    drl_ep_entry_t* entries;
    uint32_t        cap;
} drl_ep_log_t;

typedef struct {
    int32_t obs_dim;
    int32_t hidden;
    int32_t num_actions;
    int32_t obs_stride;
} drl_net_t;

typedef struct {
    float*   obs;
    uint8_t* act;
    float*   logp;
    float*   val;
    float*   rew;
    uint8_t* done;
    float*   logits;
} drl_rollout_buf_t;

typedef struct {
    float clip_coef;
    float ent_coef;
    float vf_coef;
} drl_ppo_coef_t;

#define DRL_CTRL_MAX_STEPS 64
typedef struct {
    uint64_t env_step;
    uint32_t epoch_ctr;
    uint32_t comm_seq;
    int64_t  adam_step;
    float    neg_step_size[DRL_CTRL_MAX_STEPS];
    float    bc2_sqrt[DRL_CTRL_MAX_STEPS];
} drl_ctrl_t;

int         drl_abi_version(void);
const char* drl_last_error(void);

int drl_env_obs_dim(int32_t kind);
int drl_env_num_actions(int32_t kind);
int drl_env_obs_stride(int32_t kind);
int64_t drl_param_count(const drl_net_t* net);
int64_t drl_packed_count(const drl_net_t* net);
int drl_record_width(const drl_net_t* net);
size_t drl_workspace_bytes(const drl_net_t* net);

int drl_env_reset(const drl_env_t* env, float* obs_out , void* stream);
int drl_env_observe(const drl_env_t* env, float* obs_out , void* stream);
int drl_env_step(const drl_env_t* env, uint64_t step, const int32_t* actions , float* obs_out ,
                 float* rew_out , uint8_t* done_out , const drl_ep_log_t* log, void* stream);

int drl_pack_params(const drl_net_t* net, const float* params, float* packed_out, void* stream);
int drl_policy_forward(const drl_net_t* net, const float* packed, const float* obs , int64_t n,
                       float* logits_out , float* value_out , void* stream);
int drl_sample(const float* logits , int64_t n, int32_t num_actions, uint64_t seed, uint32_t env_gid0,
               uint64_t step, int32_t* act_out , float* logp_out , void* stream);

#define DRL_ROLLOUT_TENSOR_CORES 1u
int drl_rollout(const drl_env_t* env, const drl_net_t* net, const float* packed, int32_t T, uint64_t step0,
                const drl_rollout_buf_t* buf, const drl_ep_log_t* log, uint32_t flags, void* stream);

int drl_ctrl_set(drl_ctrl_t* ctrl, uint64_t env_step, uint32_t epoch_ctr, uint32_t comm_seq, int64_t adam_step, int32_t n_steps,
                 double lr, double beta1, double beta2, void* stream);
int drl_rollout_ctl(const drl_env_t* env, const drl_net_t* net, const float* packed, int32_t T, const drl_ctrl_t* ctrl,
                    const drl_rollout_buf_t* buf, const drl_ep_log_t* log, uint32_t flags, void* stream);
int drl_permutation_ctl(uint32_t* idx_out, uint32_t B, uint64_t seed, const drl_ctrl_t* ctrl, uint32_t epoch_off, uint32_t rank,
                        void* stream);
int drl_adv_stats_perm_ctl(const drl_net_t* net, const float* adv, uint32_t B, uint32_t mb_size, uint64_t seed, const drl_ctrl_t* ctrl,
                           uint32_t epoch_off, uint32_t rank, float* stats_out, void* workspace, size_t workspace_bytes, void* stream);

int drl_gae(const drl_rollout_buf_t* buf, const drl_net_t* net, int32_t T, int32_t N, float gamma, float gae_lambda,
            float* adv_out, float* ret_out, float* rec_out, void* stream);

int drl_explained_variance(const float* values, const float* returns, int64_t n, float* out, void* workspace,
                           size_t workspace_bytes, void* stream);

int drl_permutation(uint32_t* idx_out , uint32_t B, uint64_t seed, uint32_t epoch_ctr, uint32_t rank, void* stream);

int drl_adv_stats(const drl_net_t* net, const float* rec, const uint32_t* idx, uint32_t B, uint32_t mb_size,
                  float* stats_out, void* workspace, size_t workspace_bytes, void* stream);

int drl_adv_stats_perm(const drl_net_t* net, const float* adv, uint32_t B, uint32_t mb_size, uint64_t seed, uint32_t epoch_ctr,
                       uint32_t rank, float* stats_out, void* workspace, size_t workspace_bytes, void* stream);

#define DRL_GRAD_TENSOR_CORES 1u
int drl_ppo_minibatch_grad(const drl_net_t* net, const float* packed, const float* rec, const uint32_t* idx,
                           uint32_t mb_start, uint32_t mb_count, const float* adv_stats ,
                           const drl_ppo_coef_t* coef, float* grad_out, float* loss_terms_out,
                           void* workspace, size_t workspace_bytes, uint32_t flags, void* stream);

#define DRL_MAX_RANKS 8
typedef struct {
    int32_t  world, rank;
    void*    peer[DRL_MAX_RANKS];
    uint32_t seq;
    int32_t* error_flag;
} drl_comm_t;
size_t drl_comm_bytes(const drl_net_t* net);
int drl_comm_alloc(size_t bytes, void** dev_ptr_out, void* ipc_handle_out );
int drl_comm_open(const void* ipc_handle , void** peer_ptr_out);
int drl_comm_close(void* peer_ptr);
int drl_comm_free(void* dev_ptr);

int drl_ppo_minibatch_update(const drl_net_t* net, float* packed, const float* rec, const uint32_t* idx, uint32_t mb_start,
                             uint32_t mb_count, const float* adv_stats, const drl_ppo_coef_t* coef, float* params, float* grad_out,
                             float* exp_avg, float* exp_avg_sq, int64_t step, double lr, double beta1, double beta2, double eps,
                             double max_grad_norm, float* loss_terms_out, float* norm_out, void* workspace, size_t workspace_bytes,
                             uint32_t flags, int32_t num_steps, void* stream);
int drl_ppo_minibatch_update_dist(const drl_net_t* net, float* packed, const float* rec, const uint32_t* idx, uint32_t mb_start,
                                  uint32_t mb_count, const float* adv_stats, const drl_ppo_coef_t* coef, float* params,
                                  float* grad_out, float* exp_avg, float* exp_avg_sq, int64_t step, double lr, double beta1,
                                  double beta2, double eps, double max_grad_norm, float* loss_terms_out, float* norm_out,
                                  void* workspace, size_t workspace_bytes, uint32_t flags, const drl_comm_t* comm, int32_t num_steps,
                                  void* stream);

int drl_ppo_minibatch_update_ctl(const drl_net_t* net, float* packed, const float* rec, const uint32_t* idx, uint32_t mb_start,
                                 uint32_t mb_count, const float* adv_stats, const drl_ppo_coef_t* coef, float* params,
                                 float* grad_out, float* exp_avg, float* exp_avg_sq, const drl_ctrl_t* ctrl, int32_t ordinal,
                                 double beta1, double beta2, double eps, double max_grad_norm, float* loss_terms_out,
                                 float* norm_out, void* workspace, size_t workspace_bytes, uint32_t flags, const drl_comm_t* comm,
                                 int32_t num_steps, void* stream);

int drl_clip_adam(const drl_net_t* net, float* params, const float* grad, float* exp_avg, float* exp_avg_sq,
                  int64_t step, double lr, double beta1, double beta2, double eps, double max_grad_norm,
                  double grad_scale, float* packed_out, float* norm_out, void* stream);

int drl_replay_sample_uniform(uint32_t* idx_out, uint32_t batch, uint32_t size, uint64_t seed, uint64_t draw_ctr, void* stream);
int drl_replay_gather(const float* obs, const int32_t* act, const float* rew, const uint8_t* term, const uint32_t* idx, uint32_t batch,
                      int32_t obs_stride, float* b_obs, float* b_next_obs, int32_t* b_act, float* b_rew, uint8_t* b_term, void* stream);
size_t drl_replay_scratch_bytes(uint32_t size);
int drl_replay_sample_priority(const float* priorities, uint32_t size, float alpha, uint32_t batch, uint64_t seed, uint64_t draw_ctr,
                               uint32_t* idx_out, float* prob_out, void* scratch, size_t scratch_bytes, void* stream);
int drl_replay_update_priorities(float* priorities, const uint32_t* idx, const float* td_errors, uint32_t batch, float* max_priority_inout,
                                 void* stream);

int drl_reinforce_param_count(void);
int drl_reinforce_episodes(const drl_env_t* env, const float* params, int32_t T, uint64_t step0, float* obs ,
                           uint8_t* act, float* rew, uint8_t* done, int32_t* ep_len , uint32_t* mask_bits_out,
                           const drl_ep_log_t* log, void* stream);
int drl_reinforce_grad(const float* params, const float* obs, const uint8_t* act, const float* returns, const int32_t* ep_len,
                       const uint32_t* mask_bits, int32_t N, uint64_t seed, uint32_t env_gid0, uint64_t step0, float grad_scale,
                       float* grad_out, float* loss_out, float* grad_part, float* loss_part, void* stream);
int drl_adam_step(float* params, const float* grad, float* exp_avg, float* exp_avg_sq, int64_t n, int64_t step, double lr, double beta1,
                  double beta2, double eps, void* stream);

int drl_selftest_umma(int32_t mode, int32_t variant, const float* a, const float* b, float* d_out, void* stream);
int drl_selftest_tanh(const float* x, float* y, int64_t n, void* stream);

#ifdef __cplusplus
}
#endif
#endif
```

Baseline: 543.9 million.

## Batch adv stats across epochs and cover all minibatches in one fused update launch

Adv-stats-perm now runs a 2D grid that computes per-minibatch advantage statistics for every epoch in one launch. Steps per launch go from 8 to 16, so one fused update kernel can cover every minibatch of an update. The tail prefetches params and Adam moments into shared memory with bulk async copies while the grid barrier runs, and param packing is split so the TC image can be refreshed separately. The aim is fewer launches and less global traffic between steps, at the cost of more complex synchronisation and shared-memory aliasing risk.

```diff
diff --git a/deep_rl_b200/_lib.py b/deep_rl_b200/_lib.py
--- a/deep_rl_b200/_lib.py
+++ b/deep_rl_b200/_lib.py
@@ -87,7 +87,7 @@
                                   C.POINTER(EpLogT), C.c_uint32, C.c_void_p]),
     "drl_permutation_ctl": (C.c_int, [u32p, C.c_uint32, C.c_uint64, C.c_void_p, C.c_uint32, C.c_uint32, C.c_void_p]),
     "drl_adv_stats_perm_ctl": (C.c_int, [C.POINTER(NetT), f32p, C.c_uint32, C.c_uint32, C.c_uint64, C.c_void_p, C.c_uint32, C.c_uint32,
-                                         f32p, C.c_void_p, C.c_size_t, C.c_void_p]),
+                                         C.c_uint32, f32p, C.c_void_p, C.c_size_t, C.c_void_p]),
     "drl_ppo_minibatch_update_ctl": (C.c_int, [C.POINTER(NetT), f32p, f32p, u32p, C.c_uint32, C.c_uint32, f32p, C.POINTER(PpoCoefT),
                                                f32p, f32p, f32p, f32p, C.c_void_p, C.c_int32, C.c_double, C.c_double, C.c_double,
                                                C.c_double, f32p, f32p, C.c_void_p, C.c_size_t, C.c_uint32, C.POINTER(CommT),
diff --git a/deep_rl_b200/csrc/drl_pack.cuh b/deep_rl_b200/csrc/drl_pack.cuh
--- a/deep_rl_b200/csrc/drl_pack.cuh
+++ b/deep_rl_b200/csrc/drl_pack.cuh
@@ -8,24 +8,61 @@
 int check_net(const drl_net_t* net);
 
 template <int O, int A>
-__device__ __forceinline__ void packed_store(float* __restrict__ packed, int i, float v) {
+__device__ __forceinline__ void packed_store_tc(float* __restrict__ tc, int i, float v) {
     using P = Packed<O, A>;
     const int net = i >= P::C_ACTOR ? 1 : 0;
     int r = i - net * P::C_ACTOR;
+    __nv_bfloat16* w1b = reinterpret_cast<__nv_bfloat16*>(tc + (P::TC_W1B - P::TC_W2)) + net * (2 * H * 8);
     if (r < H * O) {
         const int o = r / O, k = r % O;
-        packed[P::W1T + (net * O + k) * H + perm_pos(o)] = v;
-        packed[P::TC_W1 + (net * H + o) * P::OW + k] = __bfloat162float(__float2bfloat16_rn(v));
-        __nv_bfloat16* w1b = reinterpret_cast<__nv_bfloat16*>(packed + P::TC_W1B) + net * (2 * H * 8);
+        tc[P::TC_W1 - P::TC_W2 + (net * H + o) * P::OW + k] = __bfloat162float(__float2bfloat16_rn(v));
         w1b[o * 8 + k] = __float2bfloat16_rn(v);
         w1b[H * 8 + o * 8 + k] = __float2bfloat16_rn(v);
         return;
     }
     r -= H * O;
     if (r < H) {
+        tc[P::TC_B1 - P::TC_W2 + net * H + r] = __bfloat162float(__float2bfloat16_rn(v));
+        w1b[r * 8 + O] = __float2bfloat16_rn(v);
+        return;
+    }
+    r -= H;
+    if (r < H * H) {
+        const int o = r / H, k = r % H;
+        const int off = net * (H * H * 2) + o * 128 + ((((k >> 3) ^ (o & 7)) << 4)) + (k & 7) * 2;
+        *reinterpret_cast<__nv_bfloat16*>(reinterpret_cast<unsigned char*>(tc) + off) = __float2bfloat16_rn(v);
+        return;
+    }
+    r -= H * H;
+    if (r < H) {
+        tc[P::TC_B2 - P::TC_W2 + net * H + r] = v;
+        return;
+    }
+    r -= H;
+    const int nout = net == 0 ? A : 1;
+    if (r < nout * H) {
+        const int a = r / H, k = r % H;
+        tc[P::TC_W4 - P::TC_W2 + (net == 0 ? a : A) * H + k] = v;
+        return;
+    }
+    r -= nout * H;
+    tc[P::TC_B4 - P::TC_W2 + (net == 0 ? r : A)] = v;
+}
+
+template <int O, int A>
+__device__ __forceinline__ void packed_store(float* __restrict__ packed, int i, float v) {
+    using P = Packed<O, A>;
+    const int net = i >= P::C_ACTOR ? 1 : 0;
+    int r = i - net * P::C_ACTOR;
+    packed_store_tc<O, A>(packed + P::TC_W2, i, v);
+    if (r < H * O) {
+        const int o = r / O, k = r % O;
+        packed[P::W1T + (net * O + k) * H + perm_pos(o)] = v;
+        return;
+    }
+    r -= H * O;
+    if (r < H) {
         packed[P::B1 + net * H + perm_pos(r)] = v;
-        packed[P::TC_B1 + net * H + r] = __bfloat162float(__float2bfloat16_rn(v));
-        reinterpret_cast<__nv_bfloat16*>(packed + P::TC_W1B)[net * (2 * H * 8) + r * 8 + O] = __float2bfloat16_rn(v);
         return;
     }
     r -= H;
@@ -33,15 +70,11 @@
         const int o = r / H, k = r % H;
         packed[P::W2T + (net * H + k) * H + perm_pos(o)] = v;
         packed[P::W2P + (net * H + o) * H + perm_pos(k)] = v;
-        unsigned char* tc = reinterpret_cast<unsigned char*>(packed + P::TC_W2);
-        const int off = net * (H * H * 2) + o * 128 + ((((k >> 3) ^ (o & 7)) << 4)) + (k & 7) * 2;
-        *reinterpret_cast<__nv_bfloat16*>(tc + off) = __float2bfloat16_rn(v);
         return;
     }
     r -= H * H;
     if (r < H) {
         packed[P::B2 + net * H + perm_pos(r)] = v;
-        packed[P::TC_B2 + net * H + r] = v;
         return;
     }
     r -= H;
@@ -49,12 +82,10 @@
     if (r < nout * H) {
         const int a = r / H, k = r % H;
         packed[P::W4 + (net * A + a) * H + perm_pos(k)] = v;
-        packed[P::TC_W4 + (net == 0 ? a : A) * H + k] = v;
         return;
     }
     r -= nout * H;
     packed[P::B4 + net * A + r] = v;
-    packed[P::TC_B4 + (net == 0 ? r : A)] = v;
 }
 
 constexpr int MAX_GRAD_CTAS = 160;
diff --git a/deep_rl_b200/csrc/drl_update.cuh b/deep_rl_b200/csrc/drl_update.cuh
--- a/deep_rl_b200/csrc/drl_update.cuh
+++ b/deep_rl_b200/csrc/drl_update.cuh
@@ -3,7 +3,7 @@
 
 namespace drl {
 
-constexpr int DRL_MAX_STEPS_PER_LAUNCH = 8;
+constexpr int DRL_MAX_STEPS_PER_LAUNCH = 16;
 
 struct AdamArgs {
     float* params; const float* grad; float* m; float* v; float* packed; float* norm_out;
diff --git a/deep_rl_b200/csrc/gae_ops.cu b/deep_rl_b200/csrc/gae_ops.cu
--- a/deep_rl_b200/csrc/gae_ops.cu
+++ b/deep_rl_b200/csrc/gae_ops.cu
@@ -189,6 +189,8 @@
                                                               float* __restrict__ stats_out, double* __restrict__ partials,
                                                               uint32_t* __restrict__ counter, const drl_ctrl_t* __restrict__ ctrl) {
     if (ctrl != nullptr) epoch_ctr += ctrl->epoch_ctr;
+    epoch_ctr += blockIdx.y;
+    const uint32_t row0 = blockIdx.y * nmb;
     const uint4 k0 = philox_seeded(seed, epoch_ctr, rank, 0u, TAG_PERM);
     const uint4 k1 = philox_seeded(seed, epoch_ctr, rank, 1u, TAG_PERM);
     const uint32_t keys[8] = {k0.x, k0.y, k0.z, k0.w, k1.x, k1.y, k1.z, k1.w};
@@ -216,33 +218,33 @@
         const int which = threadIdx.x / STATS_MAX_MB, m = threadIdx.x % STATS_MAX_MB;
         double t = 0.0;
         for (int w = 0; w < 8; ++w) t += sh[which][m][w];
-        partials[((size_t)m * STAT_PARTS + blockIdx.x) * 2 + which] = t;
+        if ((uint32_t)m < nmb) partials[((size_t)(row0 + m) * STAT_PARTS + blockIdx.x) * 2 + which] = t;
     }
     __threadfence();
     __syncthreads();
     if (threadIdx.x == 0) {
         const uint32_t done = atomicAdd(counter, 1u);
-        is_last = (done == gridDim.x - 1);
+        is_last = (done == gridDim.x * gridDim.y - 1);
     }
     __syncthreads();
     if (is_last) {
         __threadfence();
-        const uint32_t k = threadIdx.x >> 5;
-        if (k < nmb) {
+        for (uint32_t row = threadIdx.x >> 5; row < gridDim.y * nmb; row += blockDim.x >> 5) {
             double ts = 0.0, tss = 0.0;
             for (uint32_t p = threadIdx.x & 31; p < gridDim.x; p += 32) {
-                ts += __ldcg(&partials[((size_t)k * STAT_PARTS + p) * 2 + 0]);
-                tss += __ldcg(&partials[((size_t)k * STAT_PARTS + p) * 2 + 1]);
+                ts += __ldcg(&partials[((size_t)row * STAT_PARTS + p) * 2 + 0]);
+                tss += __ldcg(&partials[((size_t)row * STAT_PARTS + p) * 2 + 1]);
             }
             ts = warp_sum(ts);
             tss = warp_sum(tss);
             if ((threadIdx.x & 31) == 0) {
+                const uint32_t k = row % nmb;
                 const uint32_t klo = k * mb_size, khi = min(B, klo + mb_size);
                 const double cnt = (double)(khi - klo);
                 const double mean = ts / cnt;
                 const double var = (tss - ts * mean) / (cnt - 1.0);
-                stats_out[2 * k + 0] = (float)mean;
-                stats_out[2 * k + 1] = (float)sqrt(var > 0.0 ? var : 0.0);
+                stats_out[2 * row + 0] = (float)mean;
+                stats_out[2 * row + 1] = (float)sqrt(var > 0.0 ? var : 0.0);
             }
         }
         __syncthreads();
@@ -383,7 +385,7 @@
 }
 
 static int adv_stats_perm_impl(const drl_net_t* net, const float* adv, uint32_t B, uint32_t mb_size, uint64_t seed, uint32_t epoch_ctr,
-                               uint32_t rank, float* stats_out, void* workspace, size_t workspace_bytes, void* stream,
+                               uint32_t rank, uint32_t epochs, float* stats_out, void* workspace, size_t workspace_bytes, void* stream,
                                const drl_ctrl_t* ctrl) {
     int rc = check_net(net);
     if (rc != DRL_OK) return rc;
@@ -391,6 +393,8 @@
     DRL_REQUIRE(B > 0 && mb_size > 0 && B <= 0x80000000u, "drl_adv_stats_perm: B=%u mb_size=%u", B, mb_size);
     const uint32_t nmb = (B + mb_size - 1) / mb_size;
     if (nmb > (uint32_t)STATS_MAX_MB) { set_error("drl_adv_stats_perm: %u minibatches > %d (use drl_adv_stats)", nmb, STATS_MAX_MB); return DRL_ERR_UNSUPPORTED; }
+    DRL_REQUIRE(epochs >= 1 && epochs * nmb <= (uint32_t)MAX_MINIBATCHES, "drl_adv_stats_perm: %u epochs x %u minibatches > %d rows", epochs,
+                nmb, MAX_MINIBATCHES);
     const WorkspaceLayout w = workspace_layout(drl_param_count(net));
     DRL_REQUIRE(workspace_bytes >= w.total, "drl_adv_stats_perm: workspace %zu < %zu bytes", workspace_bytes, w.total);
     uint32_t* counter = reinterpret_cast<uint32_t*>((char*)workspace + w.counters);
@@ -399,19 +403,20 @@
     while (k < 32 && (1ull << k) < (unsigned long long)B) ++k;
     uint32_t blocks = (B + 2047u) / 2048u;
     if (blocks > (uint32_t)STAT_PARTS) blocks = STAT_PARTS;
-    adv_stats_perm_kernel<<<blocks, 256, 0, as_stream(stream)>>>(adv, B, mb_size, nmb, k / 2, k - k / 2, seed, epoch_ctr, rank,
+    adv_stats_perm_kernel<<<dim3(blocks, epochs), 256, 0, as_stream(stream)>>>(adv, B, mb_size, nmb, k / 2, k - k / 2, seed, epoch_ctr, rank,
                                                                  stats_out, partials, counter, ctrl);
     DRL_LAUNCH_CHECK("adv_stats_perm_kernel");
     return DRL_OK;
 }
 int drl_adv_stats_perm(const drl_net_t* net, const float* adv, uint32_t B, uint32_t mb_size, uint64_t seed, uint32_t epoch_ctr,
                        uint32_t rank, float* stats_out, void* workspace, size_t workspace_bytes, void* stream) {
-    return adv_stats_perm_impl(net, adv, B, mb_size, seed, epoch_ctr, rank, stats_out, workspace, workspace_bytes, stream, nullptr);
+    return adv_stats_perm_impl(net, adv, B, mb_size, seed, epoch_ctr, rank, 1u, stats_out, workspace, workspace_bytes, stream, nullptr);
 }
 int drl_adv_stats_perm_ctl(const drl_net_t* net, const float* adv, uint32_t B, uint32_t mb_size, uint64_t seed, const drl_ctrl_t* ctrl,
-                           uint32_t epoch_off, uint32_t rank, float* stats_out, void* workspace, size_t workspace_bytes, void* stream) {
+                           uint32_t epoch_off, uint32_t rank, uint32_t epochs, float* stats_out, void* workspace, size_t workspace_bytes,
+                           void* stream) {
     DRL_REQUIRE(ctrl != nullptr, "drl_adv_stats_perm_ctl: ctrl is NULL");
-    return adv_stats_perm_impl(net, adv, B, mb_size, seed, epoch_off, rank, stats_out, workspace, workspace_bytes, stream, ctrl);
-}
-
-}
+    return adv_stats_perm_impl(net, adv, B, mb_size, seed, epoch_off, rank, epochs, stats_out, workspace, workspace_bytes, stream, ctrl);
+}
+
+}
diff --git a/deep_rl_b200/csrc/update_tc.cu b/deep_rl_b200/csrc/update_tc.cu
--- a/deep_rl_b200/csrc/update_tc.cu
+++ b/deep_rl_b200/csrc/update_tc.cu
@@ -24,6 +24,9 @@
     static constexpr int OFF_CTX = OFF_RED + 16 * 12 * 4;
     static constexpr int TOTAL = OFF_CTX + 512 + 1024;
     static_assert(TOTAL <= 232448, "exceeds the 227 KB of shared memory a CTA can opt in to");
+    static constexpr int PCOPY = (P::C_ALL + 3) / 4 * 4;
+    static constexpr int OFF_COPY = OFF_H1 + 9216;
+    static_assert(OFF_COPY + 4 * PCOPY * 4 <= OFF_OBS, "the tail's copies overlap the loader's ring");
 };
 
 #ifdef DRL_TC_STAMPS
@@ -52,6 +55,7 @@
     int ppad; uint32_t mb_count; float ent_coef, vf_coef;
 };
 static_assert(sizeof(TailCtx) <= 512, "TailCtx block");
+static_assert(DRL_MAX_STEPS_PER_LAUNCH == MAX_MINIBATCHES, "one launch can cover every minibatch of an update");
 
 template <int O, int A>
 __device__ __noinline__ void tc_tail_step(const TailCtx* cx, uint32_t s, uint32_t nsteps, unsigned char* sm, uint64_t* bars) {
@@ -63,7 +67,7 @@
     constexpr uint32_t BAR_TAIL = 13;
     const TailArgs& tl = cx->tl;
     const AdamArgs& ad = tl.a;
-    const int PP = ad.P;
+    constexpr int PP = P::C_ALL;
     float neg_step_size = tl.neg_step_size_s[s], bc2_sqrt = tl.bc2_sqrt_s[s];
     uint32_t seq = tl.seq + s;
     if (tl.ctrl != nullptr) {
@@ -88,8 +92,38 @@
         }
         named_bar_sync(BAR_TAIL, TC_COMPUTE);
     };
+    umma::fence_proxy_async();
     grid_barrier(tl.ctr + 0);
     TC_KSTAMP(6);
+    const bool refresh = s + 1 < nsteps;
+    float* const cw = reinterpret_cast<float*>(sm + S::OFF_COPY);
+    float* const cm = cw + S::PCOPY;
+    float* const cv = cm + S::PCOPY;
+    float* const cg = cv + S::PCOPY;
+    auto state_src = [&](int j) -> const float* { return j == 0 ? ad.params : (j == 1 ? ad.m : ad.v); };
+    const bool bulk = ((reinterpret_cast<uintptr_t>(ad.params) | reinterpret_cast<uintptr_t>(ad.m) | reinterpret_cast<uintptr_t>(ad.v)) & 15u) == 0;
+    if (refresh) {
+        constexpr uint32_t BODY = (uint32_t)(PP / 4) * 16u;
+        if (bulk) {
+            if (tid == 0) {
+                asm volatile("fence.proxy.async;" ::: "memory");
+                mbar_expect_tx(bars, 3u * BODY);
+#pragma unroll
+                for (int j = 0; j < 3; ++j)
+                    for (uint32_t off = 0; off < BODY; off += 16384u)
+                        bulk_g2s(reinterpret_cast<char*>(cw + j * S::PCOPY) + off, reinterpret_cast<const char*>(state_src(j)) + off,
+                                 BODY - off < 16384u ? BODY - off : 16384u, bars);
+            }
+            if constexpr (PP % 4 != 0) {
+                if (tid < 3 * (PP % 4)) {
+                    const int j = tid / (PP % 4), e = PP / 4 * 4 + tid % (PP % 4);
+                    cw[j * S::PCOPY + e] = __ldcg(state_src(j) + e);
+                }
+            }
+        } else {
+            for (int e = tid; e < 3 * PP; e += TC_COMPUTE) cw[e / PP * S::PCOPY + e % PP] = __ldcg(state_src(e / PP) + e % PP);
+        }
+    }
     const int chunk = (PP + nparts - 1) / nparts;
     const int p_lo = blockIdx.x * chunk, p_hi = min(PP, p_lo + chunk);
     const int pl = tid & 63, sl = tid >> 6;
@@ -170,6 +204,12 @@
     }
     sq = warp_sum(sq);
     if (lane == 0) dred[warp] = sq;
+    if (blockIdx.x == 0 && warp >= 1 && warp <= 5 && loss_terms_out != nullptr) {
+        float t = 0.f;
+        for (int c = lane; c < nparts; c += 32) t += __ldcg(cx->loss_part + c * LOSS_TERMS + (warp - 1));
+        t = warp_sum(t);
+        if (lane == 0) sbc[4 + warp - 1] = t;
+    }
     named_bar_sync(BAR_TAIL, TC_COMPUTE);
     if (tid == 0) {
         double t = 0.0;
@@ -179,9 +219,25 @@
     TC_KSTAMP(8);
     const int p_first = p_lo + tid;
     float pre_m = 0.f, pre_v = 0.f, pre_w = 0.f;
-    if (p_first < p_hi) { pre_m = ad.m[p_first]; pre_v = ad.v[p_first]; pre_w = ad.params[p_first]; }
+    if (!refresh && p_first < p_hi) { pre_m = __ldcg(ad.m + p_first); pre_v = __ldcg(ad.v + p_first); pre_w = __ldcg(ad.params + p_first); }
+    if (refresh && bulk) mbar_wait(bars, (s + 1u) & 1u);
     grid_barrier(tl.ctr + 2);
     TC_KSTAMP(9);
+    constexpr int NPT = (PP + TC_COMPUTE - 1) / TC_COMPUTE;
+    float pre_g = 0.0f;
+    if (!refresh) {
+        if (p_first < p_hi) pre_g = __ldcg(tl.grad_out + p_first);
+    } else {
+        float gv[NPT];
+#pragma unroll
+        for (int j = 0; j < NPT; ++j) {
+            const int p = tid + j * TC_COMPUTE;
+            gv[j] = p < PP ? __ldcg(tl.grad_out + p) : 0.0f;
+        }
+#pragma unroll
+        for (int j = 0; j < NPT; ++j)
+            if (tid + j * TC_COMPUTE < PP) cg[tid + j * TC_COMPUTE] = gv[j];
+    }
     if (warp == 0) {
         double tot = 0.0;
         for (int i = lane; i < nparts; i += 32) tot += __ldcg(tl.cta_sumsq + i);
@@ -192,26 +248,33 @@
             sbc[0] = cf < 1.0f ? cf : 1.0f;
             if (blockIdx.x == 0 && ad.norm_out) *ad.norm_out = norm;
         }
-    } else if (blockIdx.x == 0 && warp >= 1 && warp <= 5 && loss_terms_out != nullptr) {
-        float t = 0.f;
-        for (int c = lane; c < nparts; c += 32) t += __ldcg(cx->loss_part + c * LOSS_TERMS + (warp - 1));
-        t = warp_sum(t);
-        if (lane == 0) sbc[4 + warp - 1] = t;
     }
     named_bar_sync(BAR_TAIL, TC_COMPUTE);
     const float coef = sbc[0];
     const bool peer_lost = multi && tl.error_flag != nullptr && *reinterpret_cast<volatile int*>(tl.error_flag) != 0;
-    for (int p = p_lo + tid; p < p_hi && !peer_lost; p += TC_COMPUTE) {
-        const float gsc = (__ldcg(tl.grad_out + p) * ad.grad_scale) * coef;
-        float m, v, wgt;
-        if (p == p_first) { m = pre_m; v = pre_v; wgt = pre_w; }
-        else { m = ad.m[p]; v = ad.v[p]; wgt = ad.params[p]; }
+    float* const img = reinterpret_cast<float*>(sm + S::OFF_W);
+    auto adam = [&](int p, float g, float m, float v, float wgt) -> float {
+        const float gsc = (g * ad.grad_scale) * coef;
         m = m + ad.om_beta1 * (gsc - m);
         v = v * ad.beta2 + (ad.om_beta2 * gsc) * gsc;
         const float denom = sqrtf(v) / bc2_sqrt + ad.eps;
         wgt = wgt + (neg_step_size * m) / denom;
-        ad.m[p] = m; ad.v[p] = v; ad.params[p] = wgt;
-        if (ad.packed != nullptr) packed_store<O, A>(ad.packed, p, wgt);
+        if (p >= p_lo && p < p_hi) {
+            ad.m[p] = m; ad.v[p] = v; ad.params[p] = wgt;
+            if (ad.packed != nullptr) packed_store<O, A>(ad.packed, p, wgt);
+        }
+        return wgt;
+    };
+    if (!peer_lost && refresh) {
+#pragma unroll 1
+        for (int p = tid; p < PP; p += TC_COMPUTE) packed_store_tc<O, A>(img, p, adam(p, cg[p], cm[p], cv[p], cw[p]));
+    } else if (!peer_lost) {
+#pragma unroll 1
+        for (int p = p_first; p < p_hi; p += TC_COMPUTE) {
+            const bool f = p == p_first;
+            adam(p, f ? pre_g : __ldcg(tl.grad_out + p), f ? pre_m : __ldcg(ad.m + p), f ? pre_v : __ldcg(ad.v + p),
+                 f ? pre_w : __ldcg(ad.params + p));
+        }
     }
     TC_KSTAMP(10);
     if (blockIdx.x == 0 && tid == 0 && loss_terms_out != nullptr) {
@@ -222,17 +285,9 @@
         loss_terms_out[4] = sbc[7] * inv; loss_terms_out[5] = sbc[8] * inv;
         loss_terms_out[6] = 0.0f; loss_terms_out[7] = 0.0f;
     }
-    if (s + 1 < nsteps) {
-        grid_barrier(tl.ctr + 1);
-        if (tid == 0) {
-            asm volatile("fence.proxy.async;" ::: "memory");
-            mbar_expect_tx(bars, (uint32_t)S::W_BYTES);
-            const char* src = reinterpret_cast<const char*>(cx->packed + P::TC_W2);
-            for (uint32_t off = 0; off < (uint32_t)S::W_BYTES; off += 16384u) {
-                const uint32_t nb = (uint32_t)S::W_BYTES - off < 16384u ? (uint32_t)S::W_BYTES - off : 16384u;
-                bulk_g2s(sm + S::OFF_W + off, src + off, nb, bars);
-            }
-        }
+    if (refresh) {
+        umma::fence_proxy_async();
+        named_bar_sync(BAR_TAIL, TC_COMPUTE);
     } else if (tid == 0) {
         __threadfence();
         if (atomicAdd(tl.ctr + 3, 1u) == gridDim.x - 1) { tl.ctr[0] = 0u; tl.ctr[1] = 0u; tl.ctr[2] = 0u; tl.ctr[3] = 0u; }
@@ -392,7 +447,7 @@
         uint32_t bc = 0;
         for (uint32_t s = 0; s < nsteps; ++s) {
         const uint32_t kbase = s * nmy;
-        mbar_wait(bars, s & 1u);
+        if (s == 0) mbar_wait(bars, 0u);
         named_bar_sync(BAR_L1, TC_THREADS);
         mbar_wait(ring_full + bn, bn_par);
         umma::fence_after_sync();
@@ -491,7 +546,7 @@
     float gb4[4] = {0.f, 0.f, 0.f, 0.f};
 
     TC_KSTAMP(1);
-    mbar_wait(bars, s & 1u);
+    if (s == 0) mbar_wait(bars, 0u);
     TC_KSTAMP(2);
 
     auto phase0 = [&](uint32_t k) {
diff --git a/deep_rl_b200/ppo.py b/deep_rl_b200/ppo.py
--- a/deep_rl_b200/ppo.py
+++ b/deep_rl_b200/ppo.py
@@ -176,10 +176,19 @@
         equal = B % cfg.minibatch_size == 0
         self.mb_per_launch = 1
         if self.grad_flags == 1 and cfg.hidden == 64 and equal and (self.world == 1 or self.peer is not None):
-            want = cfg.steps_per_launch if cfg.steps_per_launch > 0 else (self.n_mb if cfg.minibatch_size <= (1 << 19) else 1)
-            self.mb_per_launch = max(1, min(want, self.n_mb, 8))
-            while self.n_mb % self.mb_per_launch:
-                self.mb_per_launch -= 1
+            total = cfg.update_epochs * self.n_mb
+            span_ok = total <= 16 and self.n_mb <= 8 and cfg.update_epochs * B < (1 << 32)
+            small = cfg.minibatch_size <= (1 << 19)
+            want = cfg.steps_per_launch if cfg.steps_per_launch > 0 else ((total if span_ok else self.n_mb) if small else 1)
+            mb = max(1, min(want, total if span_ok else self.n_mb, 16))
+            if mb > self.n_mb:
+                while total % mb:
+                    mb -= 1
+            if mb <= self.n_mb:
+                while self.n_mb % mb:
+                    mb -= 1
+            self.mb_per_launch = mb
+        self.stats_upfront = self.mb_per_launch > self.n_mb
         self.timing = False
         self.phase_events: Dict[str, list] = {}
         self.ctrl = torch.zeros(C.sizeof(_lib.CtrlT), dtype=u8, device=dev)
@@ -250,17 +259,23 @@
         cfg = self.cfg
         B, M = cfg.batch_size, cfg.minibatch_size
         net = C.byref(self.net)
-        if self.side is not None:
+        side = self.side is not None and not self.stats_upfront
+        if side:
             self._ev_gae.record()
             self.side.wait_event(self._ev_gae)
-        with self._side():
+        with (self._side() if side else contextlib.nullcontext()):
             st = _lib.stream_ptr()
-            for epoch in range(cfg.update_epochs):
+            if ctl and self.stats_upfront:
+                with _Phase(self, "adv_stats"):
+                    _lib.check(self.L.drl_adv_stats_perm_ctl(net, self.advantages.data_ptr(), B, M, cfg.seed, self.ctrl.data_ptr(), 0,
+                                                             self.rank, cfg.update_epochs, self.adv_stats.data_ptr(),
+                                                             self.workspace.data_ptr(), self.ws_bytes, st))
+            for epoch in range(cfg.update_epochs if not (ctl and self.stats_upfront) else 0):
                 epoch_ctr = self.update_idx * cfg.update_epochs + epoch
                 with _Phase(self, "adv_stats"):
                     if ctl:
                         _lib.check(self.L.drl_adv_stats_perm_ctl(net, self.advantages.data_ptr(), B, M, cfg.seed, self.ctrl.data_ptr(), epoch,
-                                                                 self.rank, self.adv_stats[epoch].data_ptr(), self.workspace.data_ptr(),
+                                                                 self.rank, 1, self.adv_stats[epoch].data_ptr(), self.workspace.data_ptr(),
                                                                  self.ws_bytes, st))
                     elif self.n_mb <= 8:
                         _lib.check(self.L.drl_adv_stats_perm(net, self.advantages.data_ptr(), B, M, cfg.seed, epoch_ctr, self.rank,
@@ -270,14 +285,14 @@
                         _lib.check(self.L.drl_adv_stats(net, self.records.data_ptr(), self.idx[epoch].data_ptr(), B, M,
                                                         self.adv_stats[epoch].data_ptr(), self.workspace.data_ptr(),
                                                         self.ws_bytes, st))
-                if self.side is not None and not self._merge_stats:
+                if side and not self._merge_stats:
                     self._ev_stats[epoch].record()
             if self._merge_stats:
                 _dist.merge_minibatch_stats(self.adv_stats, self._mb_counts)
-                if self.side is not None:
+                if side:
                     for ev in self._ev_stats:
                         ev.record()
-        self.kernel_launches += cfg.update_epochs
+        self.kernel_launches += 1 if (ctl and self.stats_upfront) else cfg.update_epochs
 
     def optimize(self, lr: float, ctl: bool = False) -> None:
         cfg = self.cfg
@@ -291,76 +306,79 @@
         self._perms_scheduled = False
         self.schedule_adv_stats(ctl)
         st = _lib.stream_ptr()
-        for epoch in range(cfg.update_epochs):
-            if self.side is not None:
-                torch.cuda.current_stream().wait_event(self._ev_stats[epoch])
-            idx_ptr = self.idx[epoch].data_ptr()
-            stats_ptr = self.adv_stats[epoch].data_ptr()
-            for k in range(0, self.n_mb, self.mb_per_launch):
-                start = k * M
-                count = min(M, B - start)
-                row = epoch * self.n_mb + k
-                ns = self.mb_per_launch
-                if ctl:
-                    self.adam_step += ns
-                    if self.peer is not None:
-                        for _ in range(ns):
-                            self.peer.next()
-                    with _Phase(self, "minibatch_grad"):
-                        _lib.check(self.L.drl_ppo_minibatch_update_ctl(
-                            net, self.agent.packed.data_ptr(), self.records.data_ptr(), idx_ptr, start, count,
-                            stats_ptr + 8 * k, C.byref(self.coef), self.agent.flat_params.data_ptr(),
-                            self.grad.data_ptr(), self.exp_avg.data_ptr(), self.exp_avg_sq.data_ptr(), self.ctrl.data_ptr(), row,
-                            0.9, 0.999, 1e-5, cfg.max_grad_norm, self.loss_terms.data_ptr() + 32 * row,
-                            self.grad_norm.data_ptr(), self.workspace.data_ptr(), self.ws_bytes, self.grad_flags,
-                            C.byref(self.peer.struct) if self.peer is not None else None, ns, st))
-                    self.kernel_launches += 1
-                    continue
+        if self.stats_upfront and self.side is not None:
+            torch.cuda.current_stream().wait_stream(self.side)
+        if self.stats_upfront:
+            launches = [(None, self.idx.data_ptr(), self.adv_stats.data_ptr() + 8 * r, r * M, M, r)
+                        for r in range(0, cfg.update_epochs * self.n_mb, self.mb_per_launch)]
+        else:
+            launches = [(epoch, self.idx[epoch].data_ptr(), self.adv_stats[epoch].data_ptr() + 8 * k, k * M, min(M, B - k * M),
+                         epoch * self.n_mb + k)
+                        for epoch in range(cfg.update_epochs) for k in range(0, self.n_mb, self.mb_per_launch)]
+        for wait_epoch, idx_ptr, stats_ptr, start, count, row in launches:
+            if self.side is not None and wait_epoch is not None and start == 0:
+                torch.cuda.current_stream().wait_event(self._ev_stats[wait_epoch])
+            ns = self.mb_per_launch
+            if ctl:
+                self.adam_step += ns
                 if self.peer is not None:
-                    first_step = self.adam_step + 1
-                    self.adam_step += ns
-                    comm = self.peer.next()
-                    for _ in range(ns - 1):
+                    for _ in range(ns):
                         self.peer.next()
-                    comm.seq = self.peer.seq - ns + 1
-                    with _Phase(self, "minibatch_grad"):
-                        _lib.check(self.L.drl_ppo_minibatch_update_dist(
-                            net, self.agent.packed.data_ptr(), self.records.data_ptr(), idx_ptr, start, count,
-                            stats_ptr + 8 * k, C.byref(self.coef), self.agent.flat_params.data_ptr(),
-                            self.grad.data_ptr(), self.exp_avg.data_ptr(), self.exp_avg_sq.data_ptr(), first_step, lr,
-                            0.9, 0.999, 1e-5, cfg.max_grad_norm, self.loss_terms.data_ptr() + 32 * row,
-                            self.grad_norm.data_ptr(), self.workspace.data_ptr(), self.ws_bytes, self.grad_flags,
-                            C.byref(comm), ns, st))
-                    comm.seq = self.peer.seq
-                    self.kernel_launches += 1
-                    continue
-                if self.world == 1 and self.fused_step:
-                    first_step = self.adam_step + 1
-                    self.adam_step += ns
-                    with _Phase(self, "minibatch_grad"):
-                        _lib.check(self.L.drl_ppo_minibatch_update(
-                            net, self.agent.packed.data_ptr(), self.records.data_ptr(), idx_ptr, start, count,
-                            stats_ptr + 8 * k, C.byref(self.coef), self.agent.flat_params.data_ptr(),
-                            self.grad.data_ptr(), self.exp_avg.data_ptr(), self.exp_avg_sq.data_ptr(), first_step, lr,
-                            0.9, 0.999, 1e-5, cfg.max_grad_norm, self.loss_terms.data_ptr() + 32 * row,
-                            self.grad_norm.data_ptr(), self.workspace.data_ptr(), self.ws_bytes, self.grad_flags, ns, st))
-                    self.kernel_launches += 1 if self.grad_flags == 1 else 2
-                    continue
                 with _Phase(self, "minibatch_grad"):
-                    _lib.check(self.L.drl_ppo_minibatch_grad(
+                    _lib.check(self.L.drl_ppo_minibatch_update_ctl(
                         net, self.agent.packed.data_ptr(), self.records.data_ptr(), idx_ptr, start, count,
-                        stats_ptr + 8 * k, C.byref(self.coef), self.grad.data_ptr(),
-                        self.loss_terms.data_ptr() + 32 * row, self.workspace.data_ptr(), self.ws_bytes, self.grad_flags, st))
-                if self.world > 1:
-                    with _Phase(self, "allreduce"):
-                        _dist.all_reduce_sum(self.grad)
-                self.adam_step += 1
-                with _Phase(self, "clip_adam"):
-                    _lib.check(self.L.drl_clip_adam(net, self.agent.flat_params.data_ptr(), self.grad.data_ptr(),
-                                                    self.exp_avg.data_ptr(), self.exp_avg_sq.data_ptr(), self.adam_step, lr,
-                                                    0.9, 0.999, 1e-5, cfg.max_grad_norm, 1.0 / self.world,
-                                                    self.agent.packed.data_ptr(), self.grad_norm.data_ptr(), st))
-                self.kernel_launches += 3
+                        stats_ptr, C.byref(self.coef), self.agent.flat_params.data_ptr(),
+                        self.grad.data_ptr(), self.exp_avg.data_ptr(), self.exp_avg_sq.data_ptr(), self.ctrl.data_ptr(), row,
+                        0.9, 0.999, 1e-5, cfg.max_grad_norm, self.loss_terms.data_ptr() + 32 * row,
+                        self.grad_norm.data_ptr(), self.workspace.data_ptr(), self.ws_bytes, self.grad_flags,
+                        C.byref(self.peer.struct) if self.peer is not None else None, ns, st))
+                self.kernel_launches += 1
+                continue
+            if self.peer is not None:
+                first_step = self.adam_step + 1
+                self.adam_step += ns
+                comm = self.peer.next()
+                for _ in range(ns - 1):
+                    self.peer.next()
+                comm.seq = self.peer.seq - ns + 1
+                with _Phase(self, "minibatch_grad"):
+                    _lib.check(self.L.drl_ppo_minibatch_update_dist(
+                        net, self.agent.packed.data_ptr(), self.records.data_ptr(), idx_ptr, start, count,
+                        stats_ptr, C.byref(self.coef), self.agent.flat_params.data_ptr(),
+                        self.grad.data_ptr(), self.exp_avg.data_ptr(), self.exp_avg_sq.data_ptr(), first_step, lr,
+                        0.9, 0.999, 1e-5, cfg.max_grad_norm, self.loss_terms.data_ptr() + 32 * row,
+                        self.grad_norm.data_ptr(), self.workspace.data_ptr(), self.ws_bytes, self.grad_flags,
+                        C.byref(comm), ns, st))
+                comm.seq = self.peer.seq
+                self.kernel_launches += 1
+                continue
+            if self.world == 1 and self.fused_step:
+                first_step = self.adam_step + 1
+                self.adam_step += ns
+                with _Phase(self, "minibatch_grad"):
+                    _lib.check(self.L.drl_ppo_minibatch_update(
+                        net, self.agent.packed.data_ptr(), self.records.data_ptr(), idx_ptr, start, count,
+                        stats_ptr, C.byref(self.coef), self.agent.flat_params.data_ptr(),
+                        self.grad.data_ptr(), self.exp_avg.data_ptr(), self.exp_avg_sq.data_ptr(), first_step, lr,
+                        0.9, 0.999, 1e-5, cfg.max_grad_norm, self.loss_terms.data_ptr() + 32 * row,
+                        self.grad_norm.data_ptr(), self.workspace.data_ptr(), self.ws_bytes, self.grad_flags, ns, st))
+                self.kernel_launches += 1 if self.grad_flags == 1 else 2
+                continue
+            with _Phase(self, "minibatch_grad"):
+                _lib.check(self.L.drl_ppo_minibatch_grad(
+                    net, self.agent.packed.data_ptr(), self.records.data_ptr(), idx_ptr, start, count,
+                    stats_ptr, C.byref(self.coef), self.grad.data_ptr(),
+                    self.loss_terms.data_ptr() + 32 * row, self.workspace.data_ptr(), self.ws_bytes, self.grad_flags, st))
+            if self.world > 1:
+                with _Phase(self, "allreduce"):
+                    _dist.all_reduce_sum(self.grad)
+            self.adam_step += 1
+            with _Phase(self, "clip_adam"):
+                _lib.check(self.L.drl_clip_adam(net, self.agent.flat_params.data_ptr(), self.grad.data_ptr(),
+                                                self.exp_avg.data_ptr(), self.exp_avg_sq.data_ptr(), self.adam_step, lr,
+                                                0.9, 0.999, 1e-5, cfg.max_grad_norm, 1.0 / self.world,
+                                                self.agent.packed.data_ptr(), self.grad_norm.data_ptr(), st))
+            self.kernel_launches += 3
 
     def _issue_update(self, lr: float, ctl: bool) -> None:
         self.schedule_permutations(ctl)
diff --git a/include/drl_b200.h b/include/drl_b200.h
--- a/include/drl_b200.h
+++ b/include/drl_b200.h
@@ -106,7 +106,8 @@
 int drl_permutation_ctl(uint32_t* idx_out, uint32_t B, uint64_t seed, const drl_ctrl_t* ctrl, uint32_t epoch_off, uint32_t rank,
                         void* stream);
 int drl_adv_stats_perm_ctl(const drl_net_t* net, const float* adv, uint32_t B, uint32_t mb_size, uint64_t seed, const drl_ctrl_t* ctrl,
-                           uint32_t epoch_off, uint32_t rank, float* stats_out, void* workspace, size_t workspace_bytes, void* stream);
+                           uint32_t epoch_off, uint32_t rank, uint32_t epochs, float* stats_out, void* workspace, size_t workspace_bytes,
+                           void* stream);
 
 int drl_gae(const drl_rollout_buf_t* buf, const drl_net_t* net, int32_t T, int32_t N, float gamma, float gae_lambda,
             float* adv_out, float* ret_out, float* rec_out, void* stream);
```

Result: slower. 523.4 million (median of 6 runs) (-3.8%).
